# marbl/meryl

Hardware: AMD Instinct MI355X
Metric: distinct k-mers counted/sec (whole node) (higher is better)
Workload: dtype u64; 1 GPU; meryl count k=21 on synthetic short reads: 66666667 x 150 bp reads per GPU (10.00 Gbp per GPU, 30x of a 333333334 bp genome, 0.5% substitutions, 0.01% N), inputs resident in HBM; k=21, reads_per_gpu=66666667, bases_per_gpu=10066666717, n_distinct=1181289506, parallelism=1 GPU, transport=none (one GPU), n_instances=8648488363, w_prefix=18

## Files before the change

### meryl_amd/build.py

```python
import os
import shutil
import subprocess
import sys

HERE = os.path.dirname(os.path.abspath(__file__))
CSRC = os.path.join(HERE, "csrc")
LIB = os.path.join(HERE, "libmeryl_gpu_count.so")
SOURCES = ["mgc_kmer.hip", "mgc_sort.hip", "mgc_scan.hip", "mgc_finish.hip", "mgc_misc.hip", "mgc_parse.hip",
           "mgc_encode.hip", "mgc_decode.hip", "mgc_merge.hip", "mgc_merge_many.hip", "mgc_lookup.hip", "mgc_filter.hip", "mgc_import.hip", "mgc_analyze.hip", "mgc_value_hist.hip",
           "mgc_api.cpp", "mgc_textfile.cpp", "mgc_import.cpp", "mgc_analyze.cpp", "mgc_count.cpp", "mgc_stream.cpp", "mgc_eval.cpp", "mgc_runs.cpp", "mgc_node.cpp", "meryl_db.cpp", "meryl_seq.cpp"]
HEADERS = ["mgc_device.h", "mgc_common.hpp", "mdb_layout.h", "mdb_statistics.hpp", "mgc_session.hpp", "mgc_clock.hpp", "mgc_chunk_ring.hpp", "mgc_bgzf.hpp", "mgc_runs.hpp", "mgc_lookup_dev.hpp", "mgc_import_dev.hpp", "mgc_analyze_dev.hpp", "mgc_label.hpp", "mgc_selector.hpp", "mgc_value.hpp", "mgc_route.hpp",
           os.path.join("..", "..", "include", "meryl_gpu_count.h"),
           os.path.join("..", "..", "include", "meryl_db.h"), os.path.join("..", "..", "include", "meryl_seq.h"),
           os.path.join("..", "..", "include", "meryl_lookup.h"), os.path.join("..", "..", "include", "meryl_import.h"),
           os.path.join("..", "..", "include", "meryl_analyze.h")]
OBJDIR = os.path.join(HERE, "build")
CFLAGS = ["--offload-arch=gfx950", "-O3", "-std=c++17", "-fPIC", "-pthread", "-Wall", "-Wno-unused-function"]
LFLAGS = ["--offload-arch=gfx950", "-shared", "-fPIC", "-pthread", "-no-hip-rt"]


def hipcc():
    for cand in (os.environ.get("HIPCC"), shutil.which("hipcc"), "/opt/rocm/bin/hipcc"):
        if cand and os.path.exists(cand):
            return cand
    raise RuntimeError("hipcc not found: the native library cannot be built")


def _sources():
    return [f for f in SOURCES if os.path.exists(os.path.join(CSRC, f))]


def _header_mtime():
    deps = [os.path.join(CSRC, f) for f in HEADERS if os.path.exists(os.path.join(CSRC, f))]
    deps.append(os.path.abspath(__file__))
    return max(os.path.getmtime(d) for d in deps)


def _obj(f):
    return os.path.join(OBJDIR, f + ".o")


def _stale_objects(force=False):
    ht = _header_mtime()
    out = []
    for f in _sources():
        o = _obj(f)
        if force or not os.path.exists(o) or os.path.getmtime(o) < max(os.path.getmtime(os.path.join(CSRC, f)), ht):
            out.append(f)
    return out


def _stale():
    if not os.path.exists(LIB) or _stale_objects():
        return True
    t = os.path.getmtime(LIB)
    return any(os.path.getmtime(_obj(f)) > t for f in _sources())


CLI = os.path.join(HERE, "bin", "meryl")
LOOKUP_CLI = os.path.join(HERE, "bin", "meryl-lookup")
IMPORT_CLI = os.path.join(HERE, "bin", "meryl-import")
ANALYZE_CLI = os.path.join(HERE, "bin", "meryl-analyze")


def _build_front_end(source, out, force, verbose):
    src = os.path.join(CSRC, source)
    if (not force and os.path.exists(out) and os.path.getmtime(out) >= os.path.getmtime(src)
            and os.path.getmtime(out) >= os.path.getmtime(LIB)):
        return out
    os.makedirs(os.path.dirname(out), exist_ok=True)
    rocm_lib = os.path.join(os.environ.get("ROCM_PATH", "/opt/rocm"), "lib")
    tmp = "%s.tmp%d" % (out, os.getpid())
    cmd = [hipcc(), "-O2", "-std=c++17", "-pthread", src, "-o", tmp, "-L" + HERE, "-lmeryl_gpu_count",
           "-Wl,-rpath,$ORIGIN/..", "-L" + rocm_lib, "-lamdhip64", "-Wl,-rpath," + rocm_lib, "-lz"]
    if verbose:
        print(" ".join(cmd), file=sys.stderr)
    subprocess.check_call(cmd)
    os.replace(tmp, out)
    return out


def build_cli(force=False, verbose=False):
    return _build_front_end("meryl_main.cpp", CLI, force, verbose)


def build_lookup_cli(force=False, verbose=False):
    return _build_front_end("meryl_lookup_main.cpp", LOOKUP_CLI, force, verbose)


def build_import_cli(force=False, verbose=False):
    return _build_front_end("meryl_import_main.cpp", IMPORT_CLI, force, verbose)


def build_analyze_cli(force=False, verbose=False):
    return _build_front_end("meryl_analyze_main.cpp", ANALYZE_CLI, force, verbose)


def build(force=False, verbose=False):
    if not force and not _stale():
        build_cli(False, verbose)
        build_lookup_cli(False, verbose)
        build_import_cli(False, verbose)
        build_analyze_cli(False, verbose)
        return LIB
    os.makedirs(OBJDIR, exist_ok=True)
    todo = _stale_objects(force)
    procs = []
    for f in todo:
        tmp = "%s.tmp%d" % (_obj(f), os.getpid())
        cmd = [hipcc()] + CFLAGS + ["-c", os.path.join(CSRC, f), "-o", tmp]
        if verbose:
            print(" ".join(cmd), file=sys.stderr)
        procs.append((f, tmp, cmd, subprocess.Popen(cmd)))
    failed = []
    for f, tmp, cmd, p in procs:
        if p.wait() != 0:
            failed.append(f)
        else:
            os.replace(tmp, _obj(f))
    if failed:
        raise subprocess.CalledProcessError(1, "hipcc -c " + " ".join(failed))
    tmp = "%s.tmp%d" % (LIB, os.getpid())
    cmd = [hipcc()] + LFLAGS + ["-o", tmp] + [_obj(f) for f in _sources()] + ["-lz"]
    if verbose:
        print(" ".join(cmd), file=sys.stderr)
    subprocess.check_call(cmd)
    os.replace(tmp, LIB)
    build_cli(True, verbose)
    build_lookup_cli(True, verbose)
    build_import_cli(True, verbose)
    build_analyze_cli(True, verbose)
    return LIB


if __name__ == "__main__":
    print(build(force="--force" in sys.argv, verbose=True))
```

### meryl_amd/csrc/mgc_api.cpp

```cpp
#include "../../include/meryl_gpu_count.h"
#include "mgc_device.h"
#include "mgc_session.hpp"
#include "mgc_runs.hpp"
#include "mgc_selector.hpp"
#include "mgc_value.hpp"

#include <algorithm>
#include <cstdio>
#include <cstdlib>
#include <cstring>
#include <map>
#include <string>
#include <thread>
#include <vector>

namespace mgc {
std::string &thread_last_error() {
  thread_local std::string e;
  return e;
}

Switches read_switches() {
  Switches sw;
  auto off = [](const char *n) { const char *e = getenv(n); return e && e[0] == '0'; };
  auto on1 = [](const char *n) { const char *e = getenv(n); return e && e[0] == '1'; };
  auto num = [](const char *n, uint64_t d) { const char *e = getenv(n); return (e && *e) ? strtoull(e, nullptr, 10) : d; };
  sw.fine_hist = !off("MGC_FINE_HIST"); sw.hpc_msd = !off("MGC_HPC_MSD"); sw.hpc_digits = !off("MGC_HPC_DIGITS");
  sw.const_k = !off("MGC_KMER_CONST_K"); sw.narrow = !off("MGC_NARROW"); sw.wide_msd = !off("MGC_WIDE_MSD");
  sw.group_pipe = !off("MGC_GROUP_PIPE"); sw.soa5 = !off("MGC_SOA5"); sw.k96 = !off("MGC_K96"); sw.finish = !off("MGC_FINISH");
  sw.nolist = on1("MGC_FINISH_NOLIST");
  sw.finish_trace = getenv("MGC_FINISH_TRACE") != nullptr; sw.group_dbg = getenv("MGC_GROUP_DBG") != nullptr; sw.hash_dbg = getenv("MGC_HASH_DBG") != nullptr;
  { const char *e = getenv("MGC_HASH_MULTI"); sw.hash_multi = (e && *e) ? atoi(e) : -1; }
  { const char *e = getenv("MGC_HASH_STREAM"); sw.hash_stream = (e && *e) ? atoi(e) : -1; }
  sw.min_top = (uint32_t)num("MGC_FINISH_MIN_TOP", 0);
  sw.finish_target = num("MGC_FINISH_TARGET", 0);
  sw.stream_max = num("MGC_STREAM_MAX", (uint64_t)1 << 22);
  sw.bucket_bases = num("MGC_BUCKET_BASES", 0);
  sw.huge_streams = (uint32_t)num("MGC_HUGE_STREAMS", 4);
  sw.huge_slices = !off("MGC_HUGE_SLICES");
  sw.pass_stagger = (uint32_t)num("MGC_PASS_STAGGER", 0);
  return sw;
}
}
using mgc::set_err;

namespace {


uint64_t number_of_bits64(uint64_t v) {
  uint64_t b = 0;
  while (v) { b++; v >>= 1; }
  return b;
}

uint64_t expected_simple_size(uint32_t k, uint64_t n_est, uint32_t suffix_len) {
  if (2 * k - 2 * suffix_len > 42) return UINT64_MAX;
  const uint64_t low_bits  = 16;
  const uint64_t n_entries = (uint64_t)1 << (2 * k - 2 * suffix_len);
  const uint64_t exp_max   = (uint64_t)(0.004 * (double)n_est);
  const uint64_t exp_bits  = number_of_bits64(exp_max) + 1;
  const uint64_t extra     = (exp_bits < low_bits) ? 0 : (exp_bits - low_bits);
  return (n_entries * low_bits + n_entries * extra) / 8;
}

void best_prefix_size(const mgc_count_config &c, uint64_t n_est, uint64_t mem_allowed, uint32_t *best,
                      uint64_t *mem_used) {
  const uint32_t k = c.k;
  const uint32_t seg_bits = c.page_size * 8, seg_bytes = c.page_size;
  *best = 0;
  *mem_used = UINT64_MAX;
  for (uint32_t wp = 1; wp < 2 * k - 1; wp++) {
    const uint64_t n_prefix = (uint64_t)1 << wp;
    const uint64_t kpp = n_est / n_prefix + 1;
    const uint64_t kps = seg_bits / (2 * k - wp);
    const uint64_t spp = kpp / kps + 1;
    if (wp + number_of_bits64(spp) + number_of_bits64(seg_bytes) >= 64) break;
    const uint64_t struct_mem = (uint64_t)c.sizeof_count_array * n_prefix + 8 * n_prefix * spp;
    const uint64_t data_min   = n_prefix * seg_bytes;
    const uint64_t total      = struct_mem + n_prefix * spp * seg_bytes;
    if (struct_mem + data_min > mem_allowed) break;
    if ((wp > 9) && (total + (uint64_t)16 * wp * 1024 * 1024 < *mem_used)) {
      *mem_used = total;
      *best = wp;
    }
    if (total > (uint64_t)16 * *mem_used) break;
  }
}

}

extern "C" uint32_t mgc_version(void) { return (0u << 16) | 3u; }

extern "C" int mgc_configure_counting(mgc_count_config *c) {
  if (!c) return MGC_EINVAL;
  if (c->k == 0 || c->k > 64) {
    set_err(nullptr, "ERROR: Kmer size not supplied with modifier k=<kmer-size>.");
    return MGC_EINVAL;
  }
  if (c->mode < 0 || c->mode > 2) return MGC_EINVAL;
  if (c->page_size == 0) c->page_size = 4096;
  if (c->sizeof_count_array == 0) c->sizeof_count_array = 3232;

  c->use_simple = 0; c->w_prefix = 0; c->n_prefix = 0; c->w_data = 0; c->n_batches = 1; c->memory_used = 0;

  const uint64_t mem_simple = expected_simple_size(c->k, c->n_kmers_estimate, c->count_suffix_length);
  uint64_t mem_complex = UINT64_MAX;
  uint32_t best = 0, n_batches = 1;

  if (c->k > 5) {
    for (n_batches = 1; mem_complex > c->memory_allowed; n_batches++) {
      best_prefix_size(*c, c->n_kmers_estimate / n_batches, c->memory_allowed, &best, &mem_complex);
      if (n_batches > (1u << 20)) {
        set_err(nullptr, "configureCounting: no prefix size fits in %lu bytes", (unsigned long)c->memory_allowed);
        return MGC_EINVAL;
      }
    }
    c->w_prefix = best;
    c->n_prefix = (uint64_t)1 << best;
    c->w_data   = 2 * c->k - best;
  }
  if ((mem_simple < mem_complex) && (mem_simple < c->memory_allowed)) {
    c->use_simple = 1; c->memory_used = mem_simple;
  } else {
    c->use_simple = 0; c->memory_used = mem_complex;
  }
  if (c->count_suffix_length > 0) { c->use_simple = 1; c->memory_used = mem_simple; }
  c->n_batches = n_batches;
  return MGC_OK;
}

extern "C" int mgc_format_configured_line(const mgc_count_config *c, char *buf, size_t buflen) {
  if (!c || !buf) return MGC_EINVAL;
  const uint64_t m = (c->memory_used < c->memory_allowed) ? c->memory_used : c->memory_allowed;
  snprintf(buf, buflen, "Configured %s mode for %.3f GB memory per batch, and up to %u batch%s.",
           c->use_simple ? "simple" : "complex", m / 1024.0 / 1024.0 / 1024.0, c->n_batches,
           (c->n_batches == 1) ? "" : "es");
  return MGC_OK;
}

namespace {
int hip_rc(hipError_t e, const char *what) {
  if (e == hipSuccess) return MGC_OK;
  set_err(nullptr, "%s: %s", what, hipGetErrorString(e));
  return (e == hipErrorOutOfMemory) ? MGC_ENOMEM : MGC_EHIP;
}
bool key_args_ok(uint32_t k, int mode, uint32_t bucket_bits) {
  if (k == 0 || k > 64) { set_err(nullptr, "k=%u out of range (1..64)", k); return false; }
  if (mode < 0 || mode > 2) { set_err(nullptr, "bad mode %d", mode); return false; }
  if (bucket_bits > MGC_MAX_BUCKET_BITS || bucket_bits > 2 * k) { set_err(nullptr, "bad bucket_bits %u", bucket_bits); return false; }
  return true;
}
}

extern "C" size_t mgc_dev_partition_workspace_bytes(uint32_t bucket_bits) {
  return mgc::kp_workspace_bytes(bucket_bits);
}

extern "C" int mgc_dev_kmer_histogram(const uint8_t *d_bases, uint64_t n_bases, uint32_t k, int mode,
                                      uint32_t bucket_bits, uint64_t *d_bucket_counts, void *d_ws, size_t ws_bytes,
                                      void *stream) {
  if (!key_args_ok(k, mode, bucket_bits)) return MGC_EINVAL;
  if ((!d_bases && n_bases) || !d_bucket_counts || !d_ws || ws_bytes < mgc::kp_workspace_bytes(bucket_bits)) return MGC_EINVAL;
  return hip_rc(mgc::launch_kmer_histogram(d_bases, n_bases, k, mode, bucket_bits, d_bucket_counts, d_ws,
                                           (hipStream_t)stream), "kmer_histogram");
}

extern "C" int mgc_dev_kmer_partition(const uint8_t *d_bases, uint64_t n_bases, uint32_t k, int mode,
                                      uint32_t bucket_bits, const uint64_t *d_bucket_starts, void *d_keys,
                                      void *d_ws, size_t ws_bytes, void *stream) {
  if (!key_args_ok(k, mode, bucket_bits)) return MGC_EINVAL;
  if ((!d_bases && n_bases) || !d_bucket_starts || !d_ws || ws_bytes < mgc::kp_workspace_bytes(bucket_bits)) return MGC_EINVAL;
  return hip_rc(mgc::launch_kmer_partition(d_bases, n_bases, k, mode, bucket_bits, d_bucket_starts, d_keys, d_ws,
                                           (hipStream_t)stream), "kmer_partition");
}

extern "C" int mgc_dev_kmer_histogram_fine(const uint8_t *d_bases, uint64_t n_bases, uint32_t k, int mode, uint32_t bucket_bits,
                                           uint64_t *d_bucket_counts, uint64_t *d_fine_hist, void *d_ws, size_t ws_bytes, void *stream) {
  if (!key_args_ok(k, mode, bucket_bits) || !mgc::kmer_histogram_fine_bits_ok(k, bucket_bits)) return MGC_EINVAL;
  if ((!d_bases && n_bases) || !d_bucket_counts || !d_fine_hist || !d_ws || ws_bytes < mgc::kp_workspace_bytes(bucket_bits)) return MGC_EINVAL;
  const mgc::Switches sw = mgc::read_switches();
  return hip_rc(mgc::launch_kmer_histogram_fine(d_bases, n_bases, k, mode, d_bucket_counts, d_fine_hist, d_ws, (hipStream_t)stream,
                                                sw.const_k, bucket_bits), "kmer_histogram_fine");
}

extern "C" size_t mgc_dev_sort_workspace_bytes(uint64_t n) { return mgc::sort_workspace_bytes(n) + 256; }

static int dev_radix_passes(void *d_keys, void *d_alt, uint64_t n, uint32_t key_words, uint32_t begin_bit, uint32_t end_bit, void *d_ws,
                           size_t ws_bytes, int *result_in_alt, void *stream, bool group);

extern "C" int mgc_dev_radix_sort(void *d_keys, void *d_alt, uint64_t n, uint32_t key_words, uint32_t begin_bit,
                                  uint32_t end_bit, void *d_ws, size_t ws_bytes, int *result_in_alt, void *stream) {
  return dev_radix_passes(d_keys, d_alt, n, key_words, begin_bit, end_bit, d_ws, ws_bytes, result_in_alt, stream, false);
}
extern "C" int mgc_dev_radix_group(void *d_keys, void *d_alt, uint64_t n, uint32_t key_words, uint32_t begin_bit,
                                   uint32_t end_bit, void *d_ws, size_t ws_bytes, int *result_in_alt, void *stream) {
  return dev_radix_passes(d_keys, d_alt, n, key_words, begin_bit, end_bit, d_ws, ws_bytes, result_in_alt, stream, true);
}

static int dev_radix_passes(void *d_keys, void *d_alt, uint64_t n, uint32_t key_words, uint32_t begin_bit, uint32_t end_bit, void *d_ws,
                           size_t ws_bytes, int *result_in_alt, void *stream, bool group) {
  if (!result_in_alt || begin_bit > end_bit || (key_words != 1 && key_words != 2) || end_bit > 64 * key_words) return MGC_EINVAL;
  *result_in_alt = 0;
  if (n == 0 || begin_bit == end_bit) return MGC_OK;
  if (!d_keys || !d_alt || !d_ws || ws_bytes < mgc::sort_workspace_bytes(n) + 256) return MGC_EINVAL;
  mgc::SortPlan plan;
  mgc::make_sort_plan(begin_bit, end_bit, &plan);
  if (group) plan.mode = 3;
  uint32_t *d_err = reinterpret_cast<uint32_t *>(reinterpret_cast<unsigned char *>(d_ws) + mgc::sort_workspace_bytes(n));
  hipStream_t st = (hipStream_t)stream;
  hipError_t e = hipMemsetAsync(d_err, 0, 4, st);
  if (e != hipSuccess) return hip_rc(e, "radix_sort memset");
  e = mgc::launch_radix_sort(d_keys, d_alt, n, key_words, plan, d_ws, ws_bytes - 256, d_err, result_in_alt, st, nullptr);
  if (e != hipSuccess) return hip_rc(e, "radix_sort");
  uint32_t h_err = 0;
  e = hipMemcpyAsync(&h_err, d_err, 4, hipMemcpyDeviceToHost, st);
  if (e == hipSuccess) e = hipStreamSynchronize(st);
  if (e != hipSuccess) return hip_rc(e, "radix_sort sync");
  if (h_err) { set_err(nullptr, "radix sort look-back timed out"); return MGC_ETIMEOUT; }
  return MGC_OK;
}

extern "C" size_t mgc_dev_rle_workspace_bytes(uint64_t n) { return mgc::rle_workspace_bytes(n); }

extern "C" int mgc_dev_rle_count(const void *d_sorted, uint64_t n, uint32_t key_words, void *d_ws, size_t ws_bytes,
                                 uint64_t *n_distinct, void *stream) {
  if (!n_distinct || !d_ws || ws_bytes < mgc::rle_workspace_bytes(n) || (!d_sorted && n) ||
      (key_words != 1 && key_words != 2)) return MGC_EINVAL;
  hipError_t e = mgc::launch_rle_count(d_sorted, n, key_words, d_ws, (hipStream_t)stream);
  if (e != hipSuccess) return hip_rc(e, "rle_count");
  return hip_rc(mgc::rle_read_total(d_ws, n_distinct, (hipStream_t)stream), "rle_count sync");
}

extern "C" int mgc_dev_rle_emit(const void *d_sorted, uint64_t n, uint32_t key_words, void *d_ws, size_t ws_bytes,
                                void *d_unique, uint32_t *d_counts, void *stream) {
  if (!d_ws || ws_bytes < mgc::rle_workspace_bytes(n) || (n && (!d_sorted || !d_unique || !d_counts)) ||
      (key_words != 1 && key_words != 2)) return MGC_EINVAL;
  return hip_rc(mgc::launch_rle_emit(d_sorted, n, key_words, d_ws, d_unique, d_counts, (hipStream_t)stream), "rle_emit");
}

extern "C" uint32_t mgc_dev_value_hist_listed_bins(void) { return mgc::value_hist_small_bins(); }

extern "C" int mgc_dev_value_hist_listed(const uint32_t *d_values, uint64_t n, uint64_t *d_hist, uint32_t *d_big, uint64_t big_cap, void *stream,
                                         uint64_t *n_pairs, uint64_t *n_listed) {
  if ((n && !d_values) || !d_hist || !d_big || big_cap < n || !n_pairs || !n_listed) { set_err(nullptr, "mgc_dev_value_hist_listed: bad arguments"); return MGC_EINVAL; }
  hipStream_t st = (hipStream_t)stream;
  const uint32_t nsmall = mgc::value_hist_small_bins();
  std::vector<uint64_t> h_hist(nsmall + 1);
  std::map<uint64_t, uint64_t> acc;
#define VL_TRY(expr) do { hipError_t e__ = (expr); if (e__ != hipSuccess) {                                         \
    set_err(nullptr, "mgc_dev_value_hist_listed: %s -> %s", #expr, hipGetErrorString(e__)); return MGC_EHIP; } } while (0)
  VL_TRY(hipMemsetAsync(d_hist, 0, 8 * (nsmall + 1), st));
  VL_TRY(mgc::launch_value_hist(d_values, n, d_hist, d_big, big_cap, d_hist + nsmall, st));
  VL_TRY(hipMemcpyAsync(h_hist.data(), d_hist, 8 * (nsmall + 1), hipMemcpyDeviceToHost, st));
  VL_TRY(hipStreamSynchronize(st));
  std::vector<uint32_t> big(h_hist[nsmall]);
  if (!big.empty()) VL_TRY(hipMemcpy(big.data(), d_big, 4 * big.size(), hipMemcpyDeviceToHost));
#undef VL_TRY
  for (uint32_t v = 0; v < nsmall; v++) if (h_hist[v]) acc[v] += h_hist[v];
  for (uint32_t v : big) acc[v]++;
  *n_pairs = acc.size();
  *n_listed = big.size();
  return MGC_OK;
}

extern "C" int mgc_dev_block_offsets(const void *d_unique, uint64_t n_distinct, uint32_t key_words, uint32_t w_data,
                                     uint64_t n_prefix, uint64_t *d_block_start, void *stream) {
  if (!d_block_start || (key_words != 1 && key_words != 2) || w_data >= 64 * key_words || (n_distinct && !d_unique))
    return MGC_EINVAL;
  return hip_rc(mgc::launch_block_offsets(d_unique, n_distinct, key_words, w_data, n_prefix, d_block_start,
                                          (hipStream_t)stream), "block_offsets");
}

extern "C" size_t mgc_dev_merge_workspace_bytes(uint64_t na, uint64_t nb) { return mgc::merge_workspace_bytes(na, nb); }

extern "C" int mgc_dev_merge_count(const void *dA, uint64_t na, const void *dB, uint64_t nb, uint32_t key_words, int op, void *d_ws,
                                   size_t ws_bytes, uint64_t *n_out, void *stream) {
  if (!n_out || !d_ws || ws_bytes < mgc::merge_workspace_bytes(na, nb) || (na && !dA) || (nb && !dB) ||
      (key_words != 1 && key_words != 2) || op < 0 || op > MGC_MERGE_SYMMETRIC_DIFFERENCE || op == MGC_MERGE_SUBTRACT) return MGC_EINVAL;
  hipError_t e = mgc::launch_merge_count(dA, na, dB, nb, key_words, op, d_ws, (hipStream_t)stream);
  if (e != hipSuccess) return hip_rc(e, "merge_count");
  return hip_rc(mgc::merge_read_total(d_ws, n_out, (hipStream_t)stream), "merge_count sync");
}

extern "C" int mgc_dev_merge_count_values(const void *dA, const uint32_t *cA, uint64_t na, const void *dB, const uint32_t *cB, uint64_t nb,
                                          uint32_t key_words, int op, void *d_ws, size_t ws_bytes, uint64_t *n_out, void *stream) {
  if (!n_out || !d_ws || ws_bytes < mgc::merge_workspace_bytes(na, nb) || (na && (!dA || !cA)) || (nb && (!dB || !cB)) ||
      (key_words != 1 && key_words != 2) || op < 0 || op > MGC_MERGE_SYMMETRIC_DIFFERENCE) return MGC_EINVAL;
  hipError_t e = mgc::launch_merge_count(dA, na, dB, nb, key_words, op, d_ws, (hipStream_t)stream, cA, cB);
  if (e != hipSuccess) return hip_rc(e, "merge_count");
  return hip_rc(mgc::merge_read_total(d_ws, n_out, (hipStream_t)stream), "merge_count sync");
}

extern "C" size_t mgc_dev_select_workspace_bytes(uint64_t n) { return mgc::select_workspace_bytes(n); }

extern "C" int mgc_dev_select_count(const void *d_keys, const uint32_t *d_values, uint64_t n, uint32_t key_words, int value_op, uint64_t constant,
                                    void *d_ws, size_t ws_bytes, uint64_t *n_out, void *stream) {
  if (!n_out || !d_ws || ws_bytes < mgc::select_workspace_bytes(n) || (n && (!d_keys || !d_values)) || (key_words != 1 && key_words != 2) ||
      value_op < 0 || value_op > MGC_VALUE_MODULO) return MGC_EINVAL;
  hipError_t e = mgc::launch_select(false, mgc::SelectInput{d_keys, d_values, nullptr, nullptr, n, key_words}, value_op, constant, mgc::PassRule(), d_ws, nullptr, nullptr,
                                    (hipStream_t)stream);
  if (e != hipSuccess) return hip_rc(e, "select_count");
  return hip_rc(mgc::merge_read_total(d_ws, n_out, (hipStream_t)stream), "select_count sync");
}

extern "C" int mgc_dev_select_emit(const void *d_keys, const uint32_t *d_values, uint64_t n, uint32_t key_words, int value_op, uint64_t constant,
                                   void *d_ws, size_t ws_bytes, void *d_keys_out, uint32_t *d_values_out, void *stream) {
  if (!d_ws || ws_bytes < mgc::select_workspace_bytes(n) || (n && (!d_keys || !d_values)) || (key_words != 1 && key_words != 2) ||
      value_op < 0 || value_op > MGC_VALUE_MODULO) return MGC_EINVAL;
  return hip_rc(mgc::launch_select(true, mgc::SelectInput{d_keys, d_values, nullptr, nullptr, n, key_words}, value_op, constant, mgc::PassRule(), d_ws, d_keys_out,
                                   d_values_out, (hipStream_t)stream), "select_emit");
}

extern "C" int mgc_dev_merge_emit(const void *dA, const uint32_t *cA, uint64_t na, const void *dB, const uint32_t *cB, uint64_t nb,
                                  uint32_t key_words, int op, void *d_ws, size_t ws_bytes, void *d_keys_out, uint32_t *d_counts_out,
                                  void *stream) {
  if (!d_ws || ws_bytes < mgc::merge_workspace_bytes(na, nb) || (na && (!dA || !cA)) || (nb && (!dB || !cB)) ||
      (key_words != 1 && key_words != 2) || op < 0 || op > MGC_MERGE_SYMMETRIC_DIFFERENCE) return MGC_EINVAL;
  return hip_rc(mgc::launch_merge_emit(dA, cA, na, dB, cB, nb, key_words, op, d_ws, d_keys_out, d_counts_out, (hipStream_t)stream),
                "merge_emit");
}

extern "C" uint32_t mgc_dev_merge_many_tile(uint32_t key_words) { return mgc::merge_many_tile(key_words); }

static bool merge_many_args_ok(const void *const *d_keys, const uint32_t *const *d_values, const uint64_t *n, uint32_t n_inputs,
                               uint32_t key_words, int op, uint32_t min_inputs = 2) {
  if (!d_keys || !d_values || !n || n_inputs < min_inputs || n_inputs > MGC_MERGE_MANY_MAX || (key_words != 1 && key_words != 2) ||
      op < MGC_MERGE_UNION_SUM || op > MGC_MERGE_UNION) return false;
  for (uint32_t i = 0; i < n_inputs; i++)
    if ((n[i] && (!d_keys[i] || !d_values[i])) || (n[i] >> 32)) return false;
  return true;
}
// ... 910 lines not shown
```

### meryl_amd/csrc/mgc_count.cpp

```cpp
#include "mgc_session.hpp"

#include <algorithm>
#include <deque>
#include <vector>

#define TRY(expr) do { const int rc__ = (expr); if (rc__ != MGC_OK) return rc__; } while (0)

namespace {
using S = mgc_session;

struct DevBuf {
  void *p = nullptr;
  ~DevBuf() { if (p) (void)hipFree(p); }
  hipError_t alloc(size_t bytes) { return hipMalloc(&p, bytes ? bytes : 256); }
};

struct StageTimer {
  bool on;
  hipStream_t st;
  hipEvent_t ev[MGC_NUM_STAGES][2];
  bool used[MGC_NUM_STAGES];
  StageTimer(bool enable, hipStream_t s) : on(enable), st(s) {
    for (int i = 0; i < MGC_NUM_STAGES; i++) {
      used[i] = false;
      if (on) { (void)hipEventCreate(&ev[i][0]); (void)hipEventCreate(&ev[i][1]); }
    }
  }
  ~StageTimer() {
    if (on) for (int i = 0; i < MGC_NUM_STAGES; i++) { (void)hipEventDestroy(ev[i][0]); (void)hipEventDestroy(ev[i][1]); }
  }
  void begin(int i) { if (on) { (void)hipEventRecord(ev[i][0], st); used[i] = true; } }
  void end(int i)   { if (on) (void)hipEventRecord(ev[i][1], st); }
};

enum class Group : uint8_t {
  NONE,
  SORT,
  NARROW,
  WIDE,
};

struct FilePlan {
  uint64_t size = 0, start = 0;
  uint32_t top = 0;
  uint32_t top_str = 0;
  mgc::SortPlan sp{};
  Group kind = Group::NONE;
  bool hpc = false;
  bool hpc_stream = false;
  bool hpc_cand = false;
  bool hpc_mixed = false;
  bool stream = false;
  bool k96 = false;
  bool msd_ok = true;
  uint32_t tr_a = 0, tr_b = 0;
  uint64_t gbase = 0, sbase = 0, slots = 0;
  size_t nws_off = 0;
  uint32_t *cnt = nullptr;
  uint64_t maxsub = 0, nlarge = 0, nzcount = 0;
  bool fallback = false;
  uint32_t passes = 0; bool narrowed = false, k96_passes = false;
  uint64_t ngf() const { return size ? (uint64_t)1 << top : 0; }
};

uint32_t plan_bucket_bits(const mgc_count_config &c, const mgc::Switches &sw, uint64_t n_bases) {
  const uint64_t per_bucket = sw.bucket_bases ? sw.bucket_bases
                                              : (c.homopoly_compress ? 60000000ull : 180000000ull);
  const uint32_t step = c.homopoly_compress ? 2u : 1u;
  uint32_t bits = MGC_NUM_FILES_BITS;
  while (bits + step <= MGC_MAX_BUCKET_BITS && bits + step <= 2 * c.k && (n_bases >> bits) > per_bucket) bits += step;
  return bits;
}

struct CountPlan {
  const mgc_count_config &c;
  const mgc::Switches &sw;
  mgc_profile &prof;
  uint32_t kw, bucket_bits, nb, rem_bits, fine_bits;
  bool fine = false;
  bool fine_hpc = false;
  uint64_t max_bucket = 0, ng_total = 0, ns_total = 0;
  uint64_t target = 0, cap = 0, starget = 0;
  bool stream_on = false, hpc_ok = false, hpc_stream_ok = false, hpc_mixed_ok = false;
  std::vector<FilePlan> files;

  CountPlan(const mgc_count_config &c_, const mgc::Switches &sw_, mgc_profile &prof_, uint32_t kw_, uint32_t bucket_bits_)
      : c(c_), sw(sw_), prof(prof_), kw(kw_), bucket_bits(bucket_bits_), nb(1u << bucket_bits_), rem_bits(2 * c_.k - bucket_bits_),
        fine_bits(15u - bucket_bits_), files(nb) {}

  mgc::SortPlan group_plan(uint32_t low) const {
    mgc::SortPlan p;
    mgc::make_sort_plan(low, rem_bits, &p);
    if (p.mode == 0) p.mode = 3;
    return p;
  }
  void fit_split(FilePlan &x) const {
    mgc::SortPlan &fp = x.sp;
    if (!fine || fp.num_passes != 2 || fp.hpc || fp.pass_bits[1] <= fine_bits) return;
    const uint32_t t = fp.pass_bits[0] + fp.pass_bits[1];
    if (t - fine_bits > 9) { x.msd_ok = false; return; }
    fp.pass_bits[1] = fine_bits; fp.pass_bits[0] = t - fine_bits;
    fp.pass_shift[1] = fp.pass_shift[0] + fp.pass_bits[0];
  }

  void init() {
    target = mgc::finish_target_for(kw, sw); cap = mgc::finish_capacity_for(kw);
    stream_on = sw.hash_stream != 0 && kw == 1 && !c.homopoly_compress;
    starget = mgc::finish_stream_target(sw);
    hpc_ok = sw.hpc_digits && c.homopoly_compress && (rem_bits % 2 == 0) && bucket_bits >= 2;
    hpc_stream_ok = hpc_ok && sw.hash_stream != 0 && sw.hash_stream != 2 && kw == 1 && fine_hpc && nb <= 256 && sw.wide_msd &&
                    rem_bits >= 20 + 32 && mgc::finish_stream_ok(kw, rem_bits - 20, false);
    hpc_mixed_ok = hpc_stream_ok && rem_bits >= 18 + 32 && mgc::finish_stream_ok(kw, rem_bits - 18, false) && mgc::finish_uses_hash(kw, rem_bits - 18);
  }

  uint32_t plan_top(FilePlan &x) const {
    uint32_t t = 0;
    if (hpc_ok && x.size > target) {
      if (x.size <= 243ull * target && rem_bits >= 10) t = 10;
      else if (x.size <= 59049ull * target && rem_bits >= 20) t = 20;
      else if (hpc_stream_ok && x.size <= 59049ull * starget && x.size < (1ull << 30)) { t = 20; x.hpc_stream = true; }
      if (t == 20 && sw.hash_stream == 1 && hpc_stream_ok && x.size < (1ull << 30)) x.hpc_stream = true;
      if (t) x.hpc = true;
    }
    if (!x.hpc) {
      while (t < rem_bits && t < 26 && (x.size >> t) > target) t++;
      if (sw.min_top) { const uint32_t m = sw.min_top; if (x.size && t < m) t = m < rem_bits ? m : rem_bits; }
      if (stream_on && x.size) {
        uint32_t ts = 0;
        while (ts < rem_bits && ts < 26 && (x.size >> ts) > starget) ts++;
        if (sw.min_top) { const uint32_t m = sw.min_top; if (ts < m) ts = m < rem_bits ? m : rem_bits; }
        x.top_str = ts;
      }
    }
    if (c.homopoly_compress && t && !x.hpc) {
      const double scale = 1.0 / (1.0 - 0.2075);
      const uint32_t tc = (uint32_t)((double)t * scale + 0.5);
      t = tc < rem_bits ? (tc < 26 ? tc : 26) : rem_bits;
    }
    return t;
  }

  void plan_hpc_kind(FilePlan &x) {
    mgc::make_hpc_group_plan(rem_bits - x.top, x.top / 10, &x.sp);
    const bool wide = fine_hpc && nb <= 256 && x.top == 20 && (kw == 2 || rem_bits - x.top >= 32) &&
                      mgc::finish_uses_hash(kw, rem_bits - x.top) && mgc::sort_plan_wide_msd(x.sp, x.size, sw.wide_msd);
    x.kind = wide ? Group::WIDE : Group::SORT;
    if (x.hpc_stream && wide) { x.stream = true; prof.stream_files++; }
    else if (hpc_stream_ok && wide && x.top == 20 && x.size < (1ull << 30)) x.hpc_cand = true;
    if ((x.hpc_cand || (x.stream && sw.hash_stream == 1)) && hpc_mixed_ok && x.size >= 19683ull * (starget * 3 / 10) &&
        x.size <= 19683ull * starget) {
      mgc::SortPlan mp;
      mgc::make_hpc_mixed_plan(rem_bits - 18, &mp);
      x.hpc_mixed = mgc::sort_plan_wide_msd(mp, x.size, sw.wide_msd);
      if (x.hpc_mixed && sw.hash_stream == 1) { take_coarser(x); x.hpc_mixed = x.hpc_cand = false; }
    }
  }

  void plan_bit_kind(FilePlan &x) {
    x.sp = group_plan(rem_bits - x.top);
    fit_split(x);
    const uint32_t low = rem_bits - x.top;
    if (low < 32 && mgc::finish_uses_hash(kw, low) && mgc::sort_plan_narrows(x.sp, x.size, kw, sw.narrow)) x.kind = Group::NARROW;
    else if (fine && nb <= 256 && x.msd_ok && mgc::finish_uses_hash(kw, low) && mgc::sort_plan_wide_msd(x.sp, x.size, sw.wide_msd)) x.kind = Group::WIDE;
    else x.kind = Group::SORT;
    if (!x.top_str) return;
    const bool narrow = x.kind == Group::NARROW;
    uint32_t ts = x.top_str;
    const uint32_t t = x.top, max_low = narrow ? 20u : 52u;
    if (rem_bits - ts > max_low) ts = rem_bits - max_low;
    bool ok = ts >= 1 && ts <= t && ts <= 18 && (ts < t || sw.hash_stream == 1) && (narrow || (x.kind == Group::WIDE && kw == 1 && sw.hash_stream != 2)) &&
              x.size < (1ull << 32) && mgc::finish_stream_ok(kw, rem_bits - ts, narrow) && mgc::finish_uses_hash(kw, rem_bits - ts);
    if (ok) {
      const mgc::SortPlan sp = group_plan(rem_bits - ts);
      if (narrow) ok = mgc::sort_plan_narrows(sp, x.size, kw, sw.narrow);
      else {
        const bool split_ok = !(fine && sp.num_passes == 2 && sp.pass_bits[1] > fine_bits && ts - fine_bits > 9);
        ok = split_ok && mgc::sort_plan_wide_msd(sp, x.size, sw.wide_msd);
      }
    }
    x.top_str = ok ? ts : 0;
  }

  void plan_files() {
    init();
    for (FilePlan &x : files) {
      x.top = plan_top(x);
      if (x.size == 0 || x.top == 0) continue;
      if (x.hpc) plan_hpc_kind(x);
      else plan_bit_kind(x);
    }
    for (FilePlan &x : files) {
      x.slots = x.ngf();
      x.gbase = ng_total; x.sbase = ns_total;
      ng_total += x.slots;
      ns_total += x.slots ? x.slots + 1 : 0;
    }
  }

  void take_coarser(FilePlan &x) {
    if (!x.stream) { x.stream = true; prof.stream_files++; }
    if (x.top_str) {
      x.top = x.top_str;
      x.sp = group_plan(rem_bits - x.top);
      x.msd_ok = true;
      fit_split(x);
    } else if (x.hpc_mixed) {
      x.top = 18;
      mgc::make_hpc_mixed_plan(rem_bits - 18, &x.sp);
      prof.hpc_mixed_files++;
    }
  }

  int choose_probe() {
    bool any_cand = false;
    for (const FilePlan &x : files) any_cand = any_cand || x.top_str != 0 || x.hpc_cand;
    if (!any_cand) return -1;
    if (sw.hash_stream == 1) {
      for (FilePlan &x : files) if (x.top_str) take_coarser(x);
      return -1;
    }
    int probe = -1;
    uint64_t best = ~0ull;
    for (uint32_t b = 0; b < nb; b++)
      if (files[b].size >= max_bucket / 16 && files[b].size >= 4096 && files[b].size < best) { best = files[b].size; probe = (int)b; }
    return probe;
  }
  void apply_probe(uint32_t probe) {
    for (uint32_t b = 0; b < nb; b++)
      if (b != probe && (files[b].top_str || (files[b].hpc_cand && !files[b].stream))) take_coarser(files[b]);
  }

  uint32_t soa_mask(bool plain_input) const {
    bool soa = sw.soa5 && plain_input && kw == 1 && nb == 64 && fine && rem_bits > 32 && rem_bits <= 40;
    for (const FilePlan &x : files) if (x.size && !(x.kind == Group::NARROW && x.top)) soa = false;
    return soa ? (1u << (rem_bits - 32)) - 1u : 0u;
  }
  bool k96_layout(bool plain_input) {
    if (!(sw.k96 && plain_input && kw == 2 && nb == 64 && fine && rem_bits <= 96 && !c.homopoly_compress)) return false;
    bool any = false;
    for (FilePlan &x : files) if (x.size && x.kind == Group::WIDE && x.top) { x.k96 = true; any = true; prof.k96_files++; }
    return any;
  }
};

struct Count {
  mgc_session *s;
  const mgc::CountInput &in;
  hipStream_t st;
  const mgc_count_config &c;
  const mgc::Switches &sw;
  mgc_profile &prof;
  const uint32_t k, kw, bucket_bits, nb, rem_bits;
  const size_t kbytes;
  CountPlan plan;
  StageTimer tm;
  hipEvent_t ev_all[2] = {nullptr, nullptr};

  const uint8_t *d_bases;
  uint64_t n_bases, N = 0, nd = 0;
  void *part_ws = nullptr, *sort_ws = nullptr, *rle_ws = nullptr;
  uint64_t *d_counts64 = nullptr, *d_starts = nullptr;
  std::vector<uint64_t> h_meta;
  const uint64_t *d_fine = nullptr, *d_fine_hpc = nullptr;
  mgc::SortPlan full{};
  bool use_finish;
  unsigned char *X = nullptr, *Y = nullptr;
  size_t sort_ws_bytes = 0;
  uint32_t *d_err = nullptr;
  uint32_t soa_hi_mask = 0;
  static constexpr uint32_t ev_per_file = 2 * 16;
  std::vector<hipEvent_t> pass_ev;
  uint32_t sort_launch_groups = 0;

  int probe = -1;
  uint64_t *d_substart = nullptr, *d_group = nullptr, *d_stats = nullptr, *d_retrycnt = nullptr;
  uint32_t *d_large = nullptr, *d_nz = nullptr;
  const size_t hdr_bytes = mgc::sort_header_bytes();
  unsigned char *d_nws = nullptr, *d_nhdrs = nullptr;
  std::deque<DevBuf> cnt_extra;
  bool fork_huge = false, forked = false, need_join = false;
  static constexpr int NH = 1 + S::HUGE_EXTRA;
  hipStream_t hstream[NH] = {};
  unsigned char *halt[NH] = {};
  void *hws[NH] = {nullptr, nullptr, nullptr, nullptr};
  size_t hws_bytes = 0;
  int n_huge_streams = 1, huge_next = 0;
  std::vector<std::pair<hipEvent_t, hipEvent_t>> fin_ev;
  uint64_t fin_keys = 0, fin_in_bytes = 0; bool fin_narrow = false;

  Count(mgc_session *s_, const mgc::CountInput &in_, uint32_t bucket_bits_)
      : s(s_), in(in_), st(s_->stream), c(s_->cfg), sw(s_->sw), prof(s_->prof), k(c.k), kw(s_->key_words), bucket_bits(bucket_bits_),
        nb(1u << bucket_bits_), rem_bits(2 * c.k - bucket_bits_), kbytes(sizeof(uint64_t) * kw), plan(c, sw, s_->prof, kw, bucket_bits_),
        tm(s_->profiling, s_->stream), d_bases(s_->d_bases), n_bases(s_->n_bases), h_meta(2 * (size_t)nb, 0), use_finish(sw.finish) {}

  void *seg(uint32_t b) const { return X + kbytes * plan.files[b].start; }
  uint32_t low(const FilePlan &x) const { return rem_bits - x.top; }
  const uint32_t *nz_list(const FilePlan &x) const { return (4 * x.nzcount < 3 * x.ngf() && !sw.nolist) ? d_nz + x.gbase : nullptr; }
  bool msd_file(const FilePlan &x) const {
    return d_fine_hpc ? x.kind == Group::WIDE : (x.kind == Group::NARROW || x.kind == Group::WIDE) && x.msd_ok;
  }
  mgc::FinishFile finish_desc(uint32_t b, bool stream, hipStream_t fst, int hsel) const;
  void take_stats(uint32_t b) {
    const uint64_t *h = s->h_stats + 3 * (size_t)b;
    plan.files[b].maxsub = h[0]; plan.files[b].nlarge = h[1]; plan.files[b].nzcount = h[2];
  }

  int run();
  int compress_bases(); int histogram(); int buffers(); int partition(bool soa, bool k96);
  int count_full();
  int count_finish(); int finish_buffers(); int prepare_headers(); int narrow_prepare(int only, int skip);
  int probe_file(); int group_file(uint32_t b); int stats_file(uint32_t b); int group_all();
  int huge_setup(); int huge_sync_all(); int huge_join_all();
  int finish_file(uint32_t b); int oversized_streams(uint32_t b, bool *stream); int widen_back(uint32_t b, bool *unordered);
  int count_file(uint32_t b, bool stream); int fallback_file(uint32_t b, bool unordered);
  int trace_slices(); int retry(); int scan_pack(); int pack_file(uint32_t b); void finish_profile();
  int block_offsets(); void collect_profile();
};

int Count::compress_bases() {
  if (!c.homopoly_compress || !n_bases || in.keys) return MGC_OK;
  HIP_TRY(s, s->ensure(S::B_HPC, n_bases));
  HIP_TRY(s, s->ensure(S::B_HPC_WS, mgc::hpc_workspace_bytes(n_bases)));
  uint8_t *d_hpc = reinterpret_cast<uint8_t *>(s->buf[S::B_HPC].p);
  void *hws_ = s->buf[S::B_HPC_WS].p;
  HIP_TRY(s, mgc::launch_homopoly_compress(d_bases, n_bases, d_hpc, hws_, st));
  uint64_t n_out = 0;
  HIP_TRY(s, hipMemcpyAsync(&n_out, hws_, sizeof(uint64_t), hipMemcpyDeviceToHost, st));
  HIP_TRY(s, hipStreamSynchronize(st));
  d_bases = d_hpc;
  n_bases = n_out;
  return MGC_OK;
}

int Count::histogram() {
  HIP_TRY(s, s->ensure(S::B_PART_WS, mgc::kp_workspace_bytes(bucket_bits)));
  HIP_TRY(s, s->ensure(S::B_META, sizeof(uint64_t) * nb * 3));
  part_ws = s->buf[S::B_PART_WS].p;
  d_counts64 = reinterpret_cast<uint64_t *>(s->buf[S::B_META].p);
  d_starts = d_counts64 + nb;
  std::vector<uint64_t> h_counts(nb);
  const bool wide_msd_on = sw.wide_msd && !c.homopoly_compress;
  if (!in.keys) {
    tm.begin(MGC_STAGE_HISTOGRAM);
    if (n_bases >= (1u << 22) && ((kw == 1 && 2 * k - bucket_bits <= 41) || wide_msd_on) && mgc::kmer_histogram_fine_ok(k, bucket_bits, s->sfx_mask, sw)) {
      HIP_TRY(s, s->ensure(S::B_FINE, sizeof(uint64_t) << 15));
      uint64_t *fine = reinterpret_cast<uint64_t *>(s->buf[S::B_FINE].p);
      HIP_TRY(s, mgc::launch_kmer_histogram_fine(d_bases, n_bases, k, c.mode, d_counts64, fine, part_ws, st, sw.const_k));
      d_fine = fine;
    } else if (c.homopoly_compress && n_bases >= (1u << 22) && (2 * k - bucket_bits) % 2 == 0 && 2 * k - bucket_bits >= 20 &&
               sw.hpc_digits && mgc::kmer_histogram_hpc_ok(k, bucket_bits, s->sfx_mask, sw)) {
      HIP_TRY(s, s->ensure(S::B_FINE, sizeof(uint64_t) * std::max<size_t>((size_t)1 << 15, mgc::kmer_histogram_hpc_entries(bucket_bits))));
      uint64_t *fine = reinterpret_cast<uint64_t *>(s->buf[S::B_FINE].p);
      HIP_TRY(s, mgc::launch_kmer_histogram_hpc(d_bases, n_bases, k, c.mode, bucket_bits, d_counts64, fine, part_ws, st, sw.const_k));
      d_fine_hpc = fine;
    } else
    HIP_TRY(s, mgc::launch_kmer_histogram(d_bases, n_bases, k, c.mode, bucket_bits, d_counts64, part_ws, st, s->sfx_mask, s->sfx_test));
    tm.end(MGC_STAGE_HISTOGRAM);
    prof.stage_launches[MGC_STAGE_HISTOGRAM] = 1;
    HIP_TRY(s, hipMemcpyAsync(h_counts.data(), d_counts64, sizeof(uint64_t) * nb, hipMemcpyDeviceToHost, st));
    HIP_TRY(s, hipStreamSynchronize(st));
  } else {
    memcpy(h_counts.data(), in.counts, sizeof(uint64_t) * nb);
    uint64_t n_ext = 0;
    for (uint32_t b = 0; b < nb; b++) n_ext += h_counts[b];
    if (in.fine && sw.fine_hist && bucket_bits <= 8 && n_ext >= (1u << 22) && s->sfx_mask == 0 && !c.homopoly_compress &&
        2 * k >= 15 + 2 && ((kw == 1 && 2 * k - bucket_bits <= 41) || wide_msd_on))
      d_fine = in.fine;
  }
  memset(s->file_instances, 0, sizeof(s->file_instances));
  for (uint32_t b = 0; b < nb; b++) {
    plan.files[b].size = h_counts[b];
    plan.files[b].start = h_meta[b] = N;
    N += h_counts[b];
    plan.max_bucket = std::max(plan.max_bucket, h_counts[b]);
    s->file_instances[b >> (bucket_bits - MGC_NUM_FILES_BITS)] += h_counts[b];
  }
  s->n_instances = N;
  plan.fine = d_fine != nullptr;
  plan.fine_hpc = d_fine_hpc != nullptr;
  return MGC_OK;
}

int Count::buffers() {
  mgc::make_sort_plan(0, rem_bits, &full);
  const bool odd = !use_finish && (full.num_passes & 1u) != 0;
  if (!in.keys) HIP_TRY(s, s->ensure(S::B_X, kbytes * N));
  HIP_TRY(s, s->ensure(S::B_Y, kbytes * (odd ? N : plan.max_bucket)));
  X = in.keys ? reinterpret_cast<unsigned char *>(in.keys) : reinterpret_cast<unsigned char *>(s->buf[S::B_X].p);
  Y = reinterpret_cast<unsigned char *>(s->buf[S::B_Y].p);
  sort_ws_bytes = mgc::sort_workspace_bytes(plan.max_bucket) + 256;
  HIP_TRY(s, s->ensure(S::B_SORT_WS, sort_ws_bytes));
  sort_ws = s->buf[S::B_SORT_WS].p;
  d_err = reinterpret_cast<uint32_t *>(reinterpret_cast<unsigned char *>(sort_ws) + sort_ws_bytes - 256);
  HIP_TRY(s, hipMemsetAsync(d_err, 0, 32, st));
  if (s->profiling) {
    pass_ev.resize((size_t)nb * ev_per_file);
    for (auto &e : pass_ev) (void)hipEventCreate(&e);
  }
  return MGC_OK;
}

int Count::partition(bool soa, bool k96) {
  if (in.keys) return MGC_OK;
  HIP_TRY(s, hipMemcpyAsync(d_starts, h_meta.data(), sizeof(uint64_t) * nb, hipMemcpyHostToDevice, st));
  uint64_t *d_k96flags = d_starts + nb;
  if (k96) HIP_TRY(s, hipMemcpyAsync(d_k96flags, h_meta.data() + nb, sizeof(uint64_t) * nb, hipMemcpyHostToDevice, st));
  tm.begin(MGC_STAGE_PARTITION);
  HIP_TRY(s, mgc::launch_kmer_partition(d_bases, n_bases, k, c.mode, bucket_bits, d_starts, (void *)X, part_ws, st,
                                        s->sfx_mask, s->sfx_test, k96 ? d_k96flags : (soa ? d_counts64 : nullptr), sw.const_k));
  tm.end(MGC_STAGE_PARTITION);
  prof.hist_bytes = n_bases;
  prof.partition_bytes = n_bases;
  for (uint32_t b = 0; b < nb; b++) prof.partition_bytes += plan.files[b].size * (soa ? 5u : ((k96 && plan.files[b].k96) ? 12u : (uint64_t)kbytes));
  prof.stage_launches[MGC_STAGE_PARTITION] = 2;
  return MGC_OK;
}

int Count::count_full() {
  TRY(partition(false, false));
  const bool odd = (full.num_passes & 1u) != 0;
  tm.begin(MGC_STAGE_SORT);
  for (uint32_t b = 0; b < nb; b++) {
    FilePlan &x = plan.files[b];
    if (x.size == 0) continue;
    void *alt = odd ? (void *)(Y + kbytes * x.start) : (void *)Y;
    int in_alt = 0;
    hipEvent_t *pe = s->profiling ? &pass_ev[(size_t)b * ev_per_file] : nullptr;
    HIP_TRY(s, mgc::launch_radix_sort(seg(b), alt, x.size, kw, full, sort_ws, sort_ws_bytes - 256, d_err, &in_alt, st, pe));
    x.passes = full.num_passes;
    sort_launch_groups++;
  }
  tm.end(MGC_STAGE_SORT);
  void *d_sorted = odd ? (void *)Y : (void *)X;

  HIP_TRY(s, s->ensure(S::B_RLE_WS, mgc::rle_workspace_bytes(N)));
  rle_ws = s->buf[S::B_RLE_WS].p;
  tm.begin(MGC_STAGE_RLE);
  HIP_TRY(s, mgc::launch_rle_count(d_sorted, N, kw, rle_ws, st));
  HIP_TRY(s, mgc::rle_read_total(rle_ws, &nd, st));
  s->n_distinct = nd;
  HIP_TRY(s, s->ensure(S::B_UNIQUE, kbytes * nd));
  HIP_TRY(s, s->ensure(S::B_COUNTS, sizeof(uint32_t) * nd));
  s->d_unique = s->buf[S::B_UNIQUE].p;
  s->d_counts = reinterpret_cast<uint32_t *>(s->buf[S::B_COUNTS].p);
  HIP_TRY(s, mgc::launch_rle_emit(d_sorted, N, kw, rle_ws, s->d_unique, s->d_counts, st));
  tm.end(MGC_STAGE_RLE);
  prof.stage_launches[MGC_STAGE_RLE] = 3;
  return MGC_OK;
}

int Count::finish_buffers() {
  const uint64_t ng_total = plan.ng_total;
  HIP_TRY(s, s->ensure(S::B_SUBSTART, sizeof(uint64_t) * (plan.ns_total + 1)));
  HIP_TRY(s, s->ensure(S::B_GROUPS, sizeof(uint64_t) * (ng_total + 2 + 3 * (uint64_t)nb)));
  HIP_TRY(s, s->ensure(S::B_LARGE, sizeof(uint32_t) * (ng_total + 1)));
  HIP_TRY(s, s->ensure(S::B_NONEMPTY, sizeof(uint32_t) * (ng_total + 1) + sizeof(uint64_t) * 2 * ((uint64_t)nb + 1)));
  HIP_TRY(s, s->ensure(S::B_GSCAN, mgc::finish_scan_scratch_bytes(ng_total + 1)));
  HIP_TRY(s, s->ensure(S::B_RLE_WS, mgc::rle_workspace_bytes(plan.max_bucket)));
  d_substart = reinterpret_cast<uint64_t *>(s->buf[S::B_SUBSTART].p);
  d_group    = reinterpret_cast<uint64_t *>(s->buf[S::B_GROUPS].p);
  d_stats    = d_group + ng_total + 1;
  d_large    = reinterpret_cast<uint32_t *>(s->buf[S::B_LARGE].p);
  d_retrycnt = reinterpret_cast<uint64_t *>(s->buf[S::B_NONEMPTY].p) + nb + 1;
  d_nz       = reinterpret_cast<uint32_t *>(d_retrycnt + nb + 1);
  HIP_TRY(s, hipMemsetAsync(s->buf[S::B_NONEMPTY].p, 0, sizeof(uint64_t) * 2 * ((size_t)nb + 1), st));
  HIP_TRY(s, hipMemsetAsync(d_group, 0, sizeof(uint64_t) * (ng_total + 1 + 3 * (size_t)nb), st));
  rle_ws = s->buf[S::B_RLE_WS].p;
  return MGC_OK;
}

int Count::prepare_headers() {
  if ((!d_fine && !d_fine_hpc) || nb > 256) return MGC_OK;
  uint64_t on[4] = {0, 0, 0, 0};
  size_t off = 0;
  bool any = false;
  for (uint32_t b = 0; b < nb; b++) {
    FilePlan &x = plan.files[b];
    x.nws_off = off;
    if (!msd_file(x)) continue;
    any = true;
    on[b >> 6] |= 1ull << (b & 63u);
    off += ((x.kind == Group::NARROW ? mgc::narrow_scratch_bytes(x.size) : mgc::wide_scratch_bytes(x.size, kw)) + 255) / 256 * 256;
  }
  if (!any) return MGC_OK;
  HIP_TRY(s, s->ensure(S::B_SORT_HDRS, hdr_bytes * nb));
  HIP_TRY(s, s->ensure(S::B_NARROW_WS, off));
  d_nhdrs = reinterpret_cast<unsigned char *>(s->buf[S::B_SORT_HDRS].p);
  d_nws = reinterpret_cast<unsigned char *>(s->buf[S::B_NARROW_WS].p);
  if (d_fine) TRY(narrow_prepare(probe, -1));
  else HIP_TRY(s, mgc::launch_hpc_prepare(d_fine_hpc, bucket_bits, on, d_nhdrs, st));
  HIP_TRY(s, hipMemsetAsync(d_nws, 0, off, st));
  return MGC_OK;
}

int Count::narrow_prepare(int only, int skip) {
  unsigned char bits_a[256] = {0}, on[256] = {0};
  bool any = false;
  for (uint32_t b = 0; b < nb; b++) {
    if (!msd_file(plan.files[b]) || (only >= 0 && (int)b != only) || (int)b == skip) continue;
    on[b] = 1; bits_a[b] = (unsigned char)plan.files[b].sp.pass_bits[1]; any = true;
  }
  if (any) HIP_TRY(s, mgc::launch_narrow_prepare(d_fine, nb, bits_a, on, d_nhdrs, st));
  return MGC_OK;
}

int Count::group_file(uint32_t b) {
  FilePlan &x = plan.files[b];
  if (x.size == 0) return MGC_OK;
  void *src = seg(b);
  hipEvent_t *pe = s->profiling ? &pass_ev[(size_t)b * ev_per_file] : nullptr;
  switch (x.kind) {
  case Group::NONE:
    return MGC_OK;
  case Group::NARROW: {
    const bool msd = d_nhdrs && d_nws && x.msd_ok;
    HIP_TRY(s, mgc::launch_group_narrow(src, (void *)Y, x.size, x.sp, sort_ws, sort_ws_bytes - 256, d_err, d_substart + x.sbase, st, pe,
                                        msd ? (void *)(d_nhdrs + hdr_bytes * b) : nullptr, msd ? (void *)(d_nws + x.nws_off) : nullptr,
                                        &x.tr_a, &x.tr_b, soa_hi_mask, sw.group_dbg, sw.group_pipe, sw.pass_stagger));
    x.passes = 2;
    x.narrowed = true;
    break;
  }
  case Group::WIDE:
    if (d_nhdrs) {
      HIP_TRY(s, mgc::launch_group_wide(src, (void *)Y, x.size, kw, x.sp, d_err, d_substart + x.sbase, st, pe,
                                        (void *)(d_nhdrs + hdr_bytes * b), (void *)(d_nws + x.nws_off), &x.tr_a, &x.tr_b, x.k96));
      x.passes = 2;
      x.k96_passes = x.k96;
      prof.wide_msd_files++;
      break;
    }
    x.kind = Group::SORT;
    [[fallthrough]];
  case Group::SORT: {
    int in_alt = 0;
    HIP_TRY(s, mgc::launch_radix_sort(src, (void *)Y, x.size, kw, x.sp, sort_ws, sort_ws_bytes - 256, d_err, &in_alt, st, pe));
    if (in_alt) HIP_TRY(s, hipMemcpyAsync(src, Y, kbytes * x.size, hipMemcpyDeviceToDevice, st));
    x.passes = x.sp.num_passes;
    break;
  }
  }
  sort_launch_groups++;
  return MGC_OK;
}

int Count::stats_file(uint32_t b) {
  const FilePlan &x = plan.files[b];
  if (x.size == 0) return MGC_OK;
  uint64_t *ds = d_stats + 3 * (size_t)b;
  if (x.kind == Group::NARROW || x.kind == Group::WIDE)
    HIP_TRY(s, mgc::launch_subbucket_max(d_substart + x.sbase, kw, low(x), x.top, ds, d_large + x.gbase, ds + 1, d_nz + x.gbase, ds + 2, st,
                                         x.stream ? mgc::finish_stream_capacity() : 0));
  else
    HIP_TRY(s, mgc::launch_subbucket_bounds(seg(b), x.size, kw, low(x), x.top, d_substart + x.sbase, ds, d_large + x.gbase, ds + 1,
                                            d_nz + x.gbase, ds + 2, st));
  return MGC_OK;
}

int Count::probe_file() {
  const uint32_t pb = (uint32_t)probe;
  const FilePlan &x = plan.files[pb];
  TRY(group_file(pb));
  TRY(stats_file(pb));
  HIP_TRY(s, hipMemcpyAsync(s->h_stats + 3 * (size_t)pb, d_stats + 3 * (size_t)pb, sizeof(uint64_t) * 3, hipMemcpyDeviceToHost, st));
  HIP_TRY(s, hipStreamSynchronize(st));
  take_stats(pb);
  TRY(finish_file(pb));
  if (need_join) TRY(huge_join_all());
  forked = false;
  uint64_t h_pd = 0;
  HIP_TRY(s, mgc::launch_sum_u64(d_group + x.gbase, x.slots, d_group + plan.ng_total, st));
  HIP_TRY(s, hipMemcpyAsync(&h_pd, d_group + plan.ng_total, sizeof(uint64_t), hipMemcpyDeviceToHost, st));
  HIP_TRY(s, hipStreamSynchronize(st));
  const double ratio = (double)h_pd / (double)x.size;
  prof.probe_ratio = ratio;
  if (sw.finish_trace) fprintf(stderr, "[finish] probe file %u: %llu distinct of %llu k-mers (%.3f): the other files take the %s plan\n", pb,
                               (unsigned long long)h_pd, (unsigned long long)x.size, ratio, ratio <= 0.30 ? "distinct-sized" : "finer");
  if (ratio <= 0.30) plan.apply_probe(pb);
  if (d_fine && nb <= 256 && d_nhdrs) TRY(narrow_prepare(-1, probe));
  return MGC_OK;
}

int Count::group_all() {
  for (uint32_t b = 0; b < nb; b++) if ((int)b != probe) TRY(group_file(b));
  tm.end(MGC_STAGE_SORT);
  tm.begin(MGC_STAGE_RLE);
  for (uint32_t b = 0; b < nb; b++) if ((int)b != probe) TRY(stats_file(b));
  HIP_TRY(s, hipMemcpyAsync(s->h_stats, d_stats, sizeof(uint64_t) * 3 * (size_t)nb, hipMemcpyDeviceToHost, st));
  HIP_TRY(s, hipStreamSynchronize(st));
  for (uint32_t b = 0; b < nb; b++) if ((int)b != probe) take_stats(b);
  return huge_setup();
}

int Count::huge_setup() {
  uint32_t files_gigantic = 0;
  for (uint32_t b = 0; b < nb; b++) if (plan.files[b].size && s->h_stats[3 * (size_t)b + 1] != 0 && s->h_stats[3 * (size_t)b] > 16384) files_gigantic++;
  if (files_gigantic && sw.huge_slices) {
    HIP_TRY(s, s->ensure(S::B_HWS0, hws_bytes));
    hws[0] = s->buf[S::B_HWS0].p;
  }
  const int want = (int)std::min<uint64_t>((uint64_t)sw.huge_streams, (uint64_t)NH);
  if (!fork_huge || want <= 1 || files_gigantic < 2) return MGC_OK;
  for (int i = 1; i < want; i++) {
    if (!s->stream_h[i - 1] && hipStreamCreateWithFlags(&s->stream_h[i - 1], hipStreamNonBlocking) != hipSuccess) { s->stream_h[i - 1] = nullptr; (void)hipGetLastError(); }
    if (!s->stream_h[i - 1]) break;
    const int id = S::B_Y2 + (i - 1);
    HIP_TRY(s, s->ensure(id, kbytes * plan.max_bucket));
    hstream[i] = s->stream_h[i - 1];
    halt[i] = reinterpret_cast<unsigned char *>(s->buf[id].p);
    if (sw.huge_slices) { HIP_TRY(s, s->ensure(S::B_HWS0 + i, hws_bytes)); hws[i] = s->buf[S::B_HWS0 + i].p; }
    n_huge_streams = i + 1;
  }
  return MGC_OK;
}

int Count::huge_sync_all() {
  for (int i = 0; i < n_huge_streams; i++) HIP_TRY(s, hipStreamSynchronize(hstream[i]));
  return MGC_OK;
}

int Count::huge_join_all() {
  for (int i = 0; i < n_huge_streams; i++) {
    HIP_TRY(s, hipEventRecord(s->ev_join, hstream[i]));
    HIP_TRY(s, hipStreamWaitEvent(st, s->ev_join, 0));
  }
  return MGC_OK;
}

int Count::finish_file(uint32_t b) {
  FilePlan &x = plan.files[b];
  x.fallback = false;
  if (x.size == 0) return MGC_OK;
  bool stream = false, unordered = false;
  TRY(oversized_streams(b, &stream));
  if (x.nlarge > 0 && !stream && (x.k96 || x.kind == Group::NARROW)) TRY(widen_back(b, &unordered));
  if (x.kind == Group::WIDE && x.nlarge > 0 && !stream) unordered = true;
  if ((x.maxsub <= plan.cap || stream) && !unordered) return count_file(b, stream);
  return fallback_file(b, unordered);
}

int Count::oversized_streams(uint32_t b, bool *stream) {
  const FilePlan &x = plan.files[b];
  *stream = mgc::finish_uses_hash(kw, low(x)) && x.nlarge > 0;
  if (*stream && x.maxsub > sw.stream_max && kw == 2) {
    *stream = false;
  } else if (*stream && x.maxsub > sw.stream_max) {
    uint32_t h_fail[3] = {0, 0, 0};
    HIP_TRY(s, hipMemsetAsync(d_err + 4, 0, 12, st));
    HIP_TRY(s, mgc::launch_finish_probe(finish_desc(b, true, st, 0), sw.stream_max, d_err + 4));
    HIP_TRY(s, hipMemcpyAsync(h_fail, d_err + 4, 12, hipMemcpyDeviceToHost, st));
    HIP_TRY(s, hipStreamSynchronize(st));
    *stream = (h_fail[0] == 0);
    if (sw.finish_trace)
      fprintf(stderr, "[finish] bucket %u: largest sub-bucket %llu > %llu, up to %u distinct in one: %s\n", b,
              (unsigned long long)x.maxsub, (unsigned long long)sw.stream_max, h_fail[2],
              *stream ? "streamed through the hash tables" : "too many distinct: stable-sort fallback");
  } else if (sw.finish_trace && x.maxsub > plan.cap) {
    fprintf(stderr, "[finish] bucket %u: largest sub-bucket %llu > %llu: %s\n", b, (unsigned long long)x.maxsub,
            (unsigned long long)plan.cap, *stream ? "streamed through the hash tables" : "stable-sort fallback");
  }
  return MGC_OK;
}

int Count::widen_back(uint32_t b, bool *unordered) {
  FilePlan &x = plan.files[b];
  if (need_join) TRY(huge_sync_all());
  forked = false;
  if (x.k96) {
    const unsigned __int128 fb = (unsigned __int128)b << rem_bits;
    HIP_TRY(s, mgc::launch_widen_k96(seg(b), x.size, (uint64_t)fb, (uint64_t)(fb >> 64), (void *)Y, st));
  } else {
    HIP_TRY(s, mgc::launch_widen_groups(seg(b), d_substart + x.sbase, x.ngf(), (uint64_t)b << rem_bits, low(x), (void *)Y, st, x.tr_a, x.tr_b));
  }
  HIP_TRY(s, hipMemcpyAsync(seg(b), Y, kbytes * x.size, hipMemcpyDeviceToDevice, st));
  if (x.k96) {
    x.k96 = false;
    prof.k96_widened_files++;
    return MGC_OK;
  }
  x.kind = Group::SORT;
  *unordered = x.tr_a != 0;
  if (x.stream) { x.stream = false; *unordered = true; }
  cnt_extra.emplace_back();
  HIP_TRY(s, cnt_extra.back().alloc(sizeof(uint32_t) * x.size));
  x.cnt = reinterpret_cast<uint32_t *>(cnt_extra.back().p);
  return MGC_OK;
}

mgc::FinishFile Count::finish_desc(uint32_t b, bool stream, hipStream_t fst, int hsel) const {
  const FilePlan &x = plan.files[b];
  mgc::FinishFile f;
  f.keys = seg(b); f.alt = halt[hsel];
  f.layout = x.kind == Group::NARROW ? mgc::FinishKeys::NARROW32 : x.k96 ? mgc::FinishKeys::K96 : kw == 2 ? mgc::FinishKeys::WHOLE16 : mgc::FinishKeys::WHOLE8;
  f.starts = d_substart + x.sbase; f.ng = x.ngf(); f.low_bits = low(x); f.tr_a = x.tr_a; f.tr_b = x.tr_b;
  f.n_keys = x.size; f.max_sub = x.maxsub;
  f.cnt_tmp = x.cnt; f.group_distinct = d_group + x.gbase;
  f.large_list = d_large + x.gbase; f.n_large = x.nlarge; f.stream = stream;
  f.nonempty_list = nz_list(x); f.nonempty_count = d_stats + 3 * (size_t)b + 2;
  f.retry_list = x.stream ? d_large + x.gbase + x.nlarge : d_nz + x.gbase; f.retry_count = d_retrycnt + b;
  f.stream_cap = x.stream ? mgc::finish_stream_capacity() : 0;
  f.huge_ws = hws[hsel]; f.huge_ws_bytes = hws_bytes; f.huge_ws_keys = plan.max_bucket; f.d_error = d_err;
  f.st = fst; f.st_huge = hstream[hsel];
  f.hash_multi = sw.hash_multi; f.hash_dbg = sw.hash_dbg;
  return f;
}

int Count::count_file(uint32_t b, bool stream) {
  const FilePlan &x = plan.files[b];
  const bool on_second = fork_huge && (b & 1u);
  if ((stream || on_second) && fork_huge && !forked) {
    HIP_TRY(s, hipEventRecord(s->ev_fork, st));
    for (int i = 0; i < n_huge_streams; i++) HIP_TRY(s, hipStreamWaitEvent(hstream[i], s->ev_fork, 0));
    forked = need_join = true;
  }
  hipStream_t fst = on_second ? s->stream2 : st;
// ... 225 lines not shown
```

### meryl_amd/csrc/mgc_device.h

```cpp
#pragma once

#include <hip/hip_runtime.h>
#include <stddef.h>
#include <stdint.h>
#include "mgc_label.hpp"
#include "../../include/meryl_gpu_count.h"

namespace mgc {

struct Switches {
  bool fine_hist = true;
  bool hpc_msd = true;
  bool hpc_digits = true;
  bool const_k = true;
  bool narrow = true;
  bool wide_msd = true;
  bool soa5 = true;
  bool group_pipe = true;
  bool k96 = true;
  bool finish = true;
  bool nolist = false;
  bool finish_trace = false;
  bool group_dbg = false;
  uint32_t pass_stagger = 0;
  bool hash_dbg = false;
  int  hash_multi = -1;
  int  hash_stream = -1;
  uint32_t min_top = 0;
  uint64_t finish_target = 0;
  uint64_t stream_max = (uint64_t)1 << 22;
  bool     huge_slices = true;
  uint32_t huge_streams = 4;
  uint64_t bucket_bases = 0;
};
Switches read_switches();



constexpr int      KP_BLOCK       = 256;
constexpr int      KP_ITEMS       = 16;
constexpr int      KP_TILE        = KP_BLOCK * KP_ITEMS;
constexpr int      KP_MAX_BUCKETS = 1024;

uint32_t kp_grid_size(uint64_t n_bases, uint32_t bucket_bits);
size_t   kp_workspace_bytes(uint32_t bucket_bits);

bool       kmer_histogram_fine_ok(uint32_t k, uint32_t bucket_bits, uint64_t sfx_mask, const Switches &sw);
bool       kmer_histogram_hpc_ok(uint32_t k, uint32_t bucket_bits, uint64_t sfx_mask, const Switches &sw);
uint32_t   kmer_histogram_hpc_entries(uint32_t bucket_bits);
hipError_t launch_kmer_histogram_hpc(const uint8_t *d_bases, uint64_t n_bases, uint32_t k, int mode, uint32_t bucket_bits,
                                     uint64_t *d_bucket_counts, uint64_t *d_fine_hist, void *d_ws, hipStream_t st, bool const_k = true );
hipError_t launch_kmer_histogram_fine(const uint8_t *d_bases, uint64_t n_bases, uint32_t k, int mode, uint64_t *d_bucket_counts,
                                      uint64_t *d_fine_hist, void *d_ws, hipStream_t st, bool const_k = true ,
                                      uint32_t bucket_bits = 6 );
bool       kmer_histogram_fine_bits_ok(uint32_t k, uint32_t bucket_bits);
hipError_t launch_kmer_histogram(const uint8_t *d_bases, uint64_t n_bases, uint32_t k, int mode,
                                 uint32_t bucket_bits, uint64_t *d_bucket_counts, void *d_ws, hipStream_t st,
                                 uint64_t sfx_mask = 0, uint64_t sfx_test = 0);
hipError_t launch_kmer_partition(const uint8_t *d_bases, uint64_t n_bases, uint32_t k, int mode,
                                 uint32_t bucket_bits, const uint64_t *d_bucket_starts, void *d_keys,
                                 void *d_ws, hipStream_t st, uint64_t sfx_mask = 0, uint64_t sfx_test = 0,
                                 const uint64_t *d_soa_counts = nullptr ,
                                 bool const_k = true );

struct SortPlan {
  uint32_t radix_bits;
  uint32_t block;
  uint32_t kpt;
  uint32_t tile;
  uint32_t mode;
  uint32_t hpc;
  uint32_t num_passes;
  uint32_t pass_shift[16];
  uint32_t pass_bits[16];
};

void   make_sort_plan(uint32_t begin_bit, uint32_t end_bit, SortPlan *plan);
void   make_hpc_group_plan(uint32_t low_bit, uint32_t passes, SortPlan *plan);
void   make_hpc_mixed_plan(uint32_t low_bit, SortPlan *plan);
size_t sort_workspace_bytes(uint64_t n);

hipError_t launch_radix_sort(void *d_keys, void *d_alt, uint64_t n, uint32_t key_words, const SortPlan &plan,
                             void *d_ws, size_t ws_bytes, uint32_t *d_error, int *result_in_alt,
                             hipStream_t st, hipEvent_t *pass_events );
size_t     sort_header_bytes();
bool       sort_plan_narrows(const SortPlan &plan, uint64_t n, uint32_t key_words, bool on = true );
size_t     narrow_scratch_bytes(uint64_t n);
hipError_t launch_narrow_prepare(const uint64_t *d_fine, uint32_t nb, const unsigned char *bits_a, const unsigned char *on, void *d_hdrs,
                                 hipStream_t st);
hipError_t launch_group_narrow(void *d_keys, void *d_alt, uint64_t n, const SortPlan &plan, void *d_ws, size_t ws_bytes,
                               uint32_t *d_error, uint64_t *d_sub_starts, hipStream_t st, hipEvent_t *pass_events ,
                               void *d_prepared, void *d_scratch, uint32_t *tr_a, uint32_t *tr_b,
                               uint32_t soa_hi_mask = 0 ,
                               bool group_dbg = false ,
                               bool pipe = true ,
                               uint32_t stagger = 0 );

bool       sort_plan_wide_msd(const SortPlan &plan, uint64_t n, bool on = true );
hipError_t launch_hpc_prepare(const uint64_t *d_fine_hpc, uint32_t bucket_bits, const uint64_t on[4], void *d_hdrs, hipStream_t st);
size_t     wide_scratch_bytes(uint64_t n, uint32_t key_words);
hipError_t launch_group_wide(void *d_keys, void *d_alt, uint64_t n, uint32_t key_words, const SortPlan &plan, uint32_t *d_error,
                             uint64_t *d_sub_starts, hipStream_t st, hipEvent_t *pass_events , void *d_prepared,
                             void *d_scratch, uint32_t *tr_a, uint32_t *tr_b,
                             bool k96 = false );

size_t     rle_workspace_bytes(uint64_t n);
hipError_t launch_rle_count(const void *d_sorted, uint64_t n, uint32_t key_words, void *d_ws, hipStream_t st);
hipError_t rle_read_total(const void *d_ws, uint64_t *n_distinct, hipStream_t st);
hipError_t launch_rle_emit(const void *d_sorted, uint64_t n, uint32_t key_words, void *d_ws, void *d_unique,
                           uint32_t *d_counts, hipStream_t st, const uint64_t *d_out_base = nullptr);

uint64_t   finish_capacity_for(uint32_t key_words);
uint64_t   finish_target_for(uint32_t key_words, const Switches &sw);
bool       finish_stream_ok(uint32_t key_words, uint32_t low_bits, bool narrow = true);
uint64_t   finish_stream_capacity();
uint64_t   finish_stream_target(const Switches &sw);
uint64_t   finish_stream_distinct();
hipError_t launch_subbucket_bounds(const void *d_keys, uint64_t n, uint32_t key_words, uint32_t low, uint32_t top_bits,
                                   uint64_t *d_starts , uint64_t *d_max ,
                                   uint32_t *d_large_list ,
                                   uint64_t *d_large_count ,
                                   uint32_t *d_nonempty_list , uint64_t *d_nonempty_count ,
                                   hipStream_t st);
hipError_t launch_subbucket_max(const uint64_t *d_starts, uint32_t key_words, uint32_t low, uint32_t top_bits, uint64_t *d_max,
                                uint32_t *d_large_list, uint64_t *d_large_count, uint32_t *d_nonempty_list, uint64_t *d_nonempty_count,
                                hipStream_t st, uint64_t small_cap = 0 );
bool       finish_uses_hash(uint32_t key_words, uint32_t low_bits);
enum class FinishKeys : uint32_t {
  WHOLE8,
  NARROW32,
  K96,
  WHOLE16,
};
struct FinishFile {
  void *keys = nullptr;
  void *alt = nullptr;
  FinishKeys layout = FinishKeys::WHOLE8;
  const uint64_t *starts = nullptr;
  uint64_t ng = 0;
  uint32_t low_bits = 0;
  uint32_t tr_a = 0, tr_b = 0;
  uint64_t n_keys = 0;
  uint64_t max_sub = 0;
  uint32_t *cnt_tmp = nullptr;
  uint64_t *group_distinct = nullptr;
  const uint32_t *large_list = nullptr;
  uint64_t n_large = 0;
  bool stream = false;
  const uint32_t *nonempty_list = nullptr;
  const uint64_t *nonempty_count = nullptr;
  uint32_t *retry_list = nullptr;
  uint64_t *retry_count = nullptr;
  uint64_t stream_cap = 0;
  void *huge_ws = nullptr; size_t huge_ws_bytes = 0; uint64_t huge_ws_keys = 0;
  uint32_t *d_error = nullptr;
  hipStream_t st = nullptr;
  hipStream_t st_huge = nullptr;
  int  hash_multi = -1;
  bool hash_dbg = false;
};
hipError_t launch_finish_probe(const FinishFile &f, uint64_t stream_max , uint32_t *d_file_fail);
hipError_t launch_finish_file(const FinishFile &f);
hipError_t launch_finish_retry(const FinishFile &f, uint64_t n_retry);
size_t     finish_huge_workspace_bytes(uint64_t n_keys);
struct HugeTrace { uint32_t cut, slices, dense; };
hipError_t finish_huge_trace(const void *d_ws, uint64_t ws_keys, HugeTrace *out);
size_t     finish_scan_scratch_bytes(uint64_t ng_total);
hipError_t launch_finish_scan(uint64_t *d_group , uint64_t ng_total, void *d_scratch, hipStream_t st);
hipError_t launch_compact_groups(const void *d_keys, uint32_t key_words, const uint32_t *d_cnt_tmp, const uint64_t *d_starts,
                                 const uint64_t *d_offs, uint64_t ng, void *d_out_keys, uint32_t *d_out_counts, hipStream_t st,
                                 uint32_t tr_a = 0, uint32_t tr_b = 0 ,
                                 const uint32_t *d_nonempty_list = nullptr, uint64_t n_nonempty = 0 );
hipError_t launch_compact_groups_narrow(const void *d_keys32, const uint32_t *d_cnt_tmp, const uint64_t *d_starts, const uint64_t *d_offs,
                                        uint64_t ng, uint64_t base, uint32_t low_bits, void *d_out_keys, uint32_t *d_out_counts, hipStream_t st,
                                        uint32_t tr_a, uint32_t tr_b, const uint32_t *d_nonempty_list = nullptr, uint64_t n_nonempty = 0);
hipError_t launch_compact_groups_k96(const void *d_keys96, const uint32_t *d_cnt_tmp, const uint64_t *d_starts, const uint64_t *d_offs,
                                     uint64_t ng, uint64_t base_lo, uint64_t base_hi, void *d_out_keys, uint32_t *d_out_counts, hipStream_t st,
                                     uint32_t tr_a, uint32_t tr_b, const uint32_t *d_nonempty_list = nullptr, uint64_t n_nonempty = 0);
hipError_t launch_widen_k96(const void *d_keys96, uint64_t n, uint64_t base_lo, uint64_t base_hi, void *d_out128, hipStream_t st);
hipError_t launch_widen_groups(const void *d_keys32, const uint64_t *d_starts, uint64_t ng, uint64_t base, uint32_t low_bits, void *d_out64,
                               hipStream_t st, uint32_t tr_a, uint32_t tr_b);
hipError_t launch_store_u64(uint64_t *d_dst, const uint64_t *d_src, hipStream_t st);
hipError_t launch_sum_u64(const uint64_t *d_in, uint64_t n, uint64_t *d_out, hipStream_t st);

hipError_t launch_block_offsets(const void *d_unique, uint64_t n_distinct, uint32_t key_words, uint32_t w_data,
                                uint64_t n_prefix, uint64_t *d_block_start, hipStream_t st);

hipError_t launch_block_offsets_range(const void *d_keys, uint64_t n, uint32_t key_words, uint32_t w_data, uint64_t prefix_begin,
                                      uint64_t n_blocks, uint64_t n_prefix_total, uint64_t *d_rel_start, hipStream_t st);
hipError_t launch_encode_sizes(const void *d_keys, uint32_t key_words, const uint64_t *d_bs, uint64_t n_blocks, uint32_t suffix_size,
                               uint32_t label_size, uint64_t *d_blk_bytes, uint64_t *d_blk_vbase, uint32_t *d_blk_bb, hipStream_t st);
hipError_t launch_encode_chunk(const void *d_keys, const uint32_t *d_counts, uint32_t key_words, const uint64_t *d_bs,
                               const uint64_t *d_blk_pos, const uint64_t *d_blk_vbase, const uint32_t *d_blk_bb,
                               uint64_t b0, uint64_t b1, uint64_t n_kmers_chunk, uint64_t prefix_of_block0,
                               uint32_t suffix_size, uint32_t label_size, uint64_t label, void *d_img, hipStream_t st,
                               const uint64_t *d_labels = nullptr );
uint32_t   value_hist_small_bins();
hipError_t launch_value_hist(const uint32_t *d_counts, uint64_t n, uint64_t *d_hist, uint32_t *d_big_list, uint64_t big_cap,
                             uint64_t *d_big_n, hipStream_t st);

hipError_t launch_decode_blocks(const void *d_file, const void *d_blocks, uint64_t n_blocks, uint32_t suffix_size, uint32_t label_size,
                                uint32_t key_words, void *d_keys, uint32_t *d_counts, uint32_t *d_err, hipStream_t st,
                                uint64_t *d_labels = nullptr );

size_t     merge_workspace_bytes(uint64_t na, uint64_t nb);
hipError_t launch_merge_count(const void *dA, uint64_t na, const void *dB, uint64_t nb, uint32_t key_words, int op, void *d_ws,
                              hipStream_t st, const uint32_t *cA = nullptr, const uint32_t *cB = nullptr);
hipError_t merge_read_total(const void *d_ws, uint64_t *n_out, hipStream_t st);
hipError_t launch_merge_emit(const void *dA, const uint32_t *cA, uint64_t na, const void *dB, const uint32_t *cB, uint64_t nb,
                             uint32_t key_words, int op, void *d_ws, void *d_out_keys, uint32_t *d_out_counts, hipStream_t st);
struct PassRule {
  int       lop = 0;
  uint64_t  lc = 0;
  bool      select = false;
  const ::mgc_select_term *terms = nullptr;
  uint32_t  n_terms = 0, k = 0;
  int       vop = 0;
  uint64_t  vc = 0;
  int       fop = -1;
  uint64_t  fc = 0;
  uint64_t *out_labs = nullptr;
};
struct MergeManyInputs { const void *const *keys; const uint32_t *const *vals; const uint64_t *const *labs; const uint64_t *n; uint32_t count, key_words; };
uint32_t   merge_many_tile(uint32_t key_words);
size_t     merge_many_workspace_bytes(const uint64_t *n, uint32_t n_inputs, uint32_t key_words);
hipError_t launch_merge_many(bool emit, const MergeManyInputs &in, int op, const PassRule &rule, void *d_ws, void *d_out_keys,
                             uint32_t *d_out_vals, hipStream_t st);
struct SelectInput { const void *keys; const uint32_t *vals; const uint32_t *flags; const uint64_t *labs; uint64_t n; uint32_t key_words; };
size_t     select_workspace_bytes(uint64_t n);
hipError_t launch_select(bool emit, const SelectInput &in, int fop, uint64_t constant, const PassRule &rule, void *d_ws, void *d_out_keys,
                         uint32_t *d_out_vals, hipStream_t st);
hipError_t launch_fill_u32(uint32_t *d, uint64_t n, uint32_t v, hipStream_t st);
hipError_t launch_last_breaker(const uint8_t *d_bases, uint64_t n, uint64_t *d_out, hipStream_t st);

size_t     hpc_workspace_bytes(uint64_t n);
hipError_t launch_homopoly_compress(const uint8_t *d_in, uint64_t n, uint8_t *d_out, void *d_ws, hipStream_t st);

size_t     text_parse_state_bytes();
size_t     text_parse_workspace_bytes(uint64_t n);
hipError_t launch_text_parse(const uint8_t *d_text, uint64_t n, int fastq, void *d_state, void *d_ws, uint8_t *d_out, hipStream_t st);
hipError_t launch_text_file_op(void *d_state, uint8_t *d_out, int what, hipStream_t st);
hipError_t launch_text_set_len(void *d_state, uint64_t new_len, int rebase_file, hipStream_t st);

hipError_t launch_synth_reads(uint64_t seed, uint64_t genome_len, uint64_t first_read, uint64_t n_reads,
                              uint32_t read_len, uint32_t sub_rate_ppm, uint32_t n_rate_ppm,
                              uint32_t repeat_ppm, uint32_t repeat_unit, uint32_t repeat_families,
                              uint8_t *d_out, hipStream_t st);

hipError_t warm_kmer(); hipError_t warm_sort(); hipError_t warm_finish(); hipError_t warm_encode(); hipError_t warm_scan();
}
```

### meryl_amd/csrc/mgc_kmer.hip

```cpp
#include "mgc_common.hpp"

namespace mgc {


__device__ __forceinline__ u32 enc4(u32 w) {
  return (((w >> 1) & 0x03030303u) * 0x40100401u) >> 24;
}
__device__ __forceinline__ u32 zero_bytes(u32 x) {
  return ~(((x & 0x7F7F7F7Fu) + 0x7F7F7F7Fu) | x | 0x7F7F7F7Fu);
}
__device__ __forceinline__ u32 inv4(u32 w) {
  const u32 u = w & 0xDFDFDFDFu;
  const u32 ok = zero_bytes(u ^ 0x41414141u) | zero_bytes(u ^ 0x43434343u) |
                 zero_bytes(u ^ 0x47474747u) | zero_bytes(u ^ 0x54545454u);
  const u32 g = ((~ok) & 0x80808080u) >> 7;
  return ((g * 0x08040201u) >> 24) & 0xFu;
}


__device__ __forceinline__ void encode16(uint4 v, u32 &codes, u32 &inval) {
  codes = (enc4(v.x) << 24) | (enc4(v.y) << 16) | (enc4(v.z) << 8) | enc4(v.w);
  inval = (inv4(v.x) << 12) | (inv4(v.y) << 8) | (inv4(v.z) << 4) | inv4(v.w);
}

__device__ __forceinline__ u64 revcomp64(u64 f, u32 key_shift ) {
  u64 x = __brevll(f ^ 0xAAAAAAAAAAAAAAAAull);
  x = ((x >> 1) & 0x5555555555555555ull) | ((x & 0x5555555555555555ull) << 1);
  return x >> key_shift;
}

constexpr int KP_WORDS = KP_TILE / 16 + 4;

__device__ __forceinline__ void kp_stage_tile(const uint8_t *__restrict__ bases, u64 n, u64 tile0, bool aligned,
                                              u32 *s_codes, u32 *s_inval) {
  const u32 t = threadIdx.x;
  {
    u32 c, iv;
    encode16(load16(bases, tile0 + (u64)t * 16, n, aligned), c, iv);
    s_codes[t] = c; s_inval[t] = iv;
  }
  if (t < 4) {
    u32 c, iv;
    encode16(load16(bases, tile0 + (u64)KP_TILE + (u64)t * 16, n, aligned), c, iv);
    s_codes[KP_BLOCK + t] = c; s_inval[KP_BLOCK + t] = iv;
  }
}

__device__ __forceinline__ u32 kp_valid_mask(u64 I, u32 k) {
  u64 X = I;
  u32 c = 1;
  while (2 * c <= k) { X |= X << c; c *= 2; }
  if (c < k) X |= X << (k - c);
  return __brev((u32)(~X >> 48) & 0xFFFFu) >> 16;
}

__device__ __forceinline__ u32 kp_thread_kmers(const u32 *s_codes, const u32 *s_inval, u32 k, int mode,
                                               u64 (&keys)[KP_ITEMS]) {
  const u32 t = threadIdx.x;
  const u64 A = ((u64)s_codes[t] << 32) | (u64)s_codes[t + 1];
  const u64 B = (u64)s_codes[t + 2] << 32;
  const u64 I = ((u64)s_inval[t] << 48) | ((u64)s_inval[t + 1] << 32) | ((u64)s_inval[t + 2] << 16);
  const u32 key_shift = 64 - 2 * k;
  const u32 top_shift = 2 * k - 2;
  u64 r = 0;
#pragma unroll
  for (int j = 0; j < KP_ITEMS; j++) {
    const u64 top = (j == 0) ? A : ((A << (2 * j)) | (B >> (64 - 2 * j)));
    const u64 f   = top >> key_shift;
    if (j == 0) r = revcomp64(f, key_shift);
    else        r = (r >> 2) | ((((f & 3ull) ^ 2ull)) << top_shift);
    u64 key;
    if      (mode == 1) key = f;
    else if (mode == 2) key = r;
    else                key = (f < r) ? f : r;
    keys[j] = key;
  }
  return kp_valid_mask(I, k);
}

__device__ __forceinline__ u32 kp_thread_buckets(const u32 *s_codes, const u32 *s_inval, u32 k, int mode, u32 bucket_bits,
                                                 u32 (&bk)[KP_ITEMS], const u32 t = threadIdx.x) {
  const u64 A = ((u64)s_codes[t] << 32) | (u64)s_codes[t + 1];
  const u64 B = (u64)s_codes[t + 2] << 32;
  const u64 I = ((u64)s_inval[t] << 48) | ((u64)s_inval[t + 1] << 32) | ((u64)s_inval[t + 2] << 16);
  const u32 m  = (bucket_bits + 1) / 2;
  const u32 z0 = k - m;
  const u64 Z  = (z0 == 0) ? A : ((A << (2 * z0)) | (B >> (64 - 2 * z0)));
  const u64 RC = revcomp64(Z, 0);
  const u64 mmask = (1ull << (2 * m)) - 1ull;
  const u32 odd = 2 * m - bucket_bits;
#pragma unroll
  for (int j = 0; j < KP_ITEMS; j++) {
    const u32 ft = (u32)(((j == 0) ? A : (A << (2 * j))) >> (64 - bucket_bits));
    const u32 rt = (u32)((RC >> (2 * j)) & mmask) >> odd;
    bk[j] = (mode == 1) ? ft : (mode == 2) ? rt : (ft < rt ? ft : rt);
  }
  return kp_valid_mask(I, k);
}

__device__ __forceinline__ u32 kp_thread_buckets_wide(const u32 *s_codes, const u32 *s_inval, u32 k, int mode, u32 bucket_bits,
                                                      u32 (&bk)[KP_ITEMS], const u32 t) {
  const u64 A  = ((u64)s_codes[t] << 32) | (u64)s_codes[t + 1];
  const u32 m  = (bucket_bits + 1) / 2, z0 = k - m;
  const u32 q  = z0 >> 4, r = z0 & 15u;
  const u64 H  = ((u64)s_codes[t + q] << 32) | (u64)s_codes[t + q + 1];
  const u64 L  = (q + 2 <= 4) ? ((u64)s_codes[t + q + 2] << 32) : 0ull;
  const u64 Z  = r ? ((H << (2 * r)) | (L >> (64 - 2 * r))) : H;
  const u64 RC = revcomp64(Z, 0);
  const u64 mmask = (1ull << (2 * m)) - 1ull;
  const u32 odd = 2 * m - bucket_bits;
#pragma unroll
  for (int j = 0; j < KP_ITEMS; j++) {
    const u32 ft = (u32)(((j == 0) ? A : (A << (2 * j))) >> (64 - bucket_bits));
    const u32 rt = (u32)((RC >> (2 * j)) & mmask) >> odd;
    bk[j] = (mode == 1) ? ft : (mode == 2) ? rt : (ft < rt ? ft : rt);
  }
  u128 X = ((u128)s_inval[t] << 112) | ((u128)s_inval[t + 1] << 96) | ((u128)s_inval[t + 2] << 80) |
           ((u128)s_inval[t + 3] << 64) | ((u128)s_inval[t + 4] << 48);
  u32 c = 1;
  while (2 * c <= k) { X |= X << c; c *= 2; }
  if (c < k) X |= X << (k - c);
  return __brev((u32)(~X >> 112) & 0xFFFFu) >> 16;
}

__device__ __forceinline__ u32 kp_thread_kmers(const u32 *s_codes, const u32 *s_inval, u32 k, int mode,
                                               K128 (&keys)[KP_ITEMS]) {
  const u32 t = threadIdx.x;
  const u128 A = ((u128)s_codes[t] << 96) | ((u128)s_codes[t + 1] << 64) | ((u128)s_codes[t + 2] << 32) |
                 (u128)s_codes[t + 3];
  const u128 B = (u128)s_codes[t + 4] << 96;
  const u128 I = ((u128)s_inval[t] << 112) | ((u128)s_inval[t + 1] << 96) | ((u128)s_inval[t + 2] << 80) |
                 ((u128)s_inval[t + 3] << 64) | ((u128)s_inval[t + 4] << 48);
  const u32 key_shift = 128 - 2 * k;
  const u32 top_shift = 2 * k - 2;
  u32 vmask = 0;
  u128 r = 0;
#pragma unroll
  for (int j = 0; j < KP_ITEMS; j++) {
    const u128 top = (j == 0) ? A : ((A << (2 * j)) | (B >> (128 - 2 * j)));
    const u128 f   = top >> key_shift;
    if (j == 0) {
      const u128 c = f ^ (((u128)0xAAAAAAAAAAAAAAAAull << 64) | (u128)0xAAAAAAAAAAAAAAAAull);
      u64 lo = __brevll((u64)(c >> 64)), hi = __brevll((u64)c);
      lo = ((lo >> 1) & 0x5555555555555555ull) | ((lo & 0x5555555555555555ull) << 1);
      hi = ((hi >> 1) & 0x5555555555555555ull) | ((hi & 0x5555555555555555ull) << 1);
      r = (((u128)hi << 64) | (u128)lo) >> key_shift;
    } else {
      r = (r >> 2) | ((u128)(((u64)f & 3ull) ^ 2ull) << top_shift);
    }
    const bool ok = (((I << j) >> (128 - k)) == (u128)0);
    u128 key;
    if      (mode == 1) key = f;
    else if (mode == 2) key = r;
    else                key = (f < r) ? f : r;
    keys[j] = KeyOps<K128>::mk(key);
    vmask |= (ok ? 1u : 0u) << j;
  }
  return vmask;
}

template <typename K>
__device__ __forceinline__ u32 kp_suffix_filter(const K (&keys)[KP_ITEMS], u32 vmask, u64 sfx_mask, u64 sfx_test) {
  if (sfx_mask == 0) return vmask;
#pragma unroll
  for (int j = 0; j < KP_ITEMS; j++)
    if ((KeyOps<K>::low64(keys[j]) & sfx_mask) != sfx_test) vmask &= ~(1u << j);
  return vmask;
}

__device__ __forceinline__ void kp_tile_range(u64 num_tiles, u64 &t_begin, u64 &t_end, u32 vwg = blockIdx.x, u32 vgrid = gridDim.x) {
  const u64 per = (num_tiles + vgrid - 1) / vgrid;
  t_begin = (u64)vwg * per;
  t_end   = t_begin + per;
  if (t_begin > num_tiles) t_begin = num_tiles;
  if (t_end   > num_tiles) t_end   = num_tiles;
}

template <typename K>
__global__ __launch_bounds__(KP_BLOCK)
void kmer_hist_kernel(const uint8_t *__restrict__ bases, u64 n, u32 k, int mode, u32 bucket_bits,
                      u64 num_tiles, u64 *__restrict__ block_hist, u64 *__restrict__ bucket_counts, u64 sfx_mask, u64 sfx_test) {
  __shared__ u32 s_codes[KP_WORDS];
  __shared__ u32 s_inval[KP_WORDS];
  __shared__ u32 s_hist[KP_MAX_BUCKETS];

  const u32  nb = 1u << bucket_bits;
  const u32  bucket_shift = 2 * k - bucket_bits;
  const bool aligned = ((reinterpret_cast<uintptr_t>(bases) & 15) == 0);

  for (u32 b = threadIdx.x; b < nb; b += KP_BLOCK) s_hist[b] = 0;
  __syncthreads();

  u64 t_begin, t_end;
  kp_tile_range(num_tiles, t_begin, t_end);
  u32 my_count = 0;

  for (u64 tile = t_begin; tile < t_end; tile++) {
    kp_stage_tile(bases, n, tile * KP_TILE, aligned, s_codes, s_inval);
    __syncthreads();
    if (sizeof(K) == 8 && nb > 1 && 2 * k >= bucket_bits && sfx_mask == 0) {
      u32 bk[KP_ITEMS];
      const u32 vmask = kp_thread_buckets(s_codes, s_inval, k, mode, bucket_bits, bk);
#pragma unroll
      for (int j = 0; j < KP_ITEMS; j++)
        if ((vmask >> j) & 1u) atomicAdd(&s_hist[bk[j]], 1u);
    } else {
      K keys[KP_ITEMS];
      const u32 vmask = kp_suffix_filter(keys, kp_thread_kmers(s_codes, s_inval, k, mode, keys), sfx_mask, sfx_test);
      if (nb == 1) {
        my_count += __popc(vmask);
      } else {
#pragma unroll
        for (int j = 0; j < KP_ITEMS; j++)
          if ((vmask >> j) & 1u) atomicAdd(&s_hist[KeyOps<K>::bucket(keys[j], bucket_shift)], 1u);
      }
    }
    __syncthreads();
  }
  if (nb == 1) atomicAdd(&s_hist[0], my_count);
  __syncthreads();

  for (u32 b = threadIdx.x; b < nb; b += KP_BLOCK) {
    const u64 v = s_hist[b];
    block_hist[(u64)blockIdx.x * nb + b] = v;
    if (v) atomicAdd(&bucket_counts[b], v);
  }
}

constexpr int KH_NV = 4, KH_FINE_BITS = 15;

__host__ __device__ constexpr u32 hpc_table_size(int hb) { u32 t = 4; for (int i = 1; i < hb; i++) t *= 3; return t; }
template <int HB>
__device__ __forceinline__ u32 hpc_dense_rank(u32 x) {
  u32 prev = (x >> (2 * HB - 2)) & 3u, r = prev;
#pragma unroll
  for (int i = 1; i < HB; i++) {
    const u32 c = (x >> (2 * (HB - 1 - i))) & 3u;
    r = r * 3u + (c - (c > prev ? 1u : 0u));
    prev = c;
  }
  return r;
}

template <int HB, int KC = 0>
__global__ __launch_bounds__(KP_BLOCK * KH_NV)
void kmer_hist_fine_kernel(const uint8_t *__restrict__ bases, u64 n, u32 k_arg, int mode_arg, u64 num_tiles, u32 vgrid,
                           u64 *__restrict__ block_hist, u64 *__restrict__ bucket_counts, u64 *__restrict__ fine_hist,
                           u32 fbits = 6 ,
                           u32 nvp = KH_NV ) {
  const u32 k = KC ? (u32)KC : k_arg;
  const int mode = KC ? 0 : mode_arg;
  constexpr u32 TABLE = HB ? hpc_table_size(HB) : (1u << KH_FINE_BITS);
  constexpr u32 NBK = HB ? (1u << (2 * (HB - 5))) : 64u;
  constexpr u32 IDX_BITS = HB ? 2u * HB : (u32)KH_FINE_BITS;
  extern __shared__ __attribute__((aligned(16))) u32 kh_fine[];
  __shared__ u32 s_codes[2][KH_NV][KP_WORDS];
  __shared__ u32 s_inval[2][KH_NV][KP_WORDS];
  __shared__ u32 s_prev[HB ? NBK : 256u];
  __shared__ unsigned short s_r5[HB ? 4096 : 1];
  __shared__ unsigned short s_rb[HB ? NBK : 1];
  const u32 tid = threadIdx.x, v = tid >> 8, t = tid & 255u;
  if constexpr (HB > 0) {
    for (u32 i = tid; i < 4096u; i += KP_BLOCK * KH_NV) s_r5[i] = (unsigned short)hpc_digit(i);
    if (tid < NBK) s_rb[tid] = (unsigned short)(hpc_dense_rank<HB - 5>(tid) * 243u);
  }
  const bool aligned = ((reinterpret_cast<uintptr_t>(bases) & 15) == 0);
  for (u32 i = tid; i < TABLE; i += KP_BLOCK * KH_NV) kh_fine[i] = 0;
  if (tid < (HB ? NBK : 256u)) s_prev[tid] = 0;

  const u64 per = (num_tiles + vgrid - 1) / vgrid;
  for (u32 vv = 0; vv < nvp; vv++) {
    const u64 vwg = (u64)blockIdx.x * nvp + vv;
    u64 t_begin = vwg * per, t_end = t_begin + per;
    if (t_begin > num_tiles) t_begin = num_tiles;
    if (t_end > num_tiles) t_end = num_tiles;
    if (vwg >= vgrid) t_begin = t_end = num_tiles;

    uint4 cur = make_uint4(0, 0, 0, 0), halo = make_uint4(0, 0, 0, 0);
    auto fetch = [&](u64 tile) {
      if (tile >= t_end) return;
      cur = load16(bases, tile * KP_TILE + (u64)t * 16, n, aligned);
      if (t < 4) halo = load16(bases, tile * KP_TILE + (u64)KP_TILE + (u64)t * 16, n, aligned);
    };
    fetch(t_begin + v);
    __syncthreads();
    const u64 rounds = (t_end - t_begin + KH_NV - 1) / KH_NV;
    for (u64 it = 0; it < rounds; it++) {
      const u64 tile = t_begin + it * KH_NV + v;
      const u32 buf = (u32)it & 1u;
      const bool active = tile < t_end;
      if (active) {
        u32 c, iv;
        encode16(cur, c, iv);
        s_codes[buf][v][t] = c; s_inval[buf][v][t] = iv;
        if (t < 4) { encode16(halo, c, iv); s_codes[buf][v][KP_BLOCK + t] = c; s_inval[buf][v][KP_BLOCK + t] = iv; }
      }
      __syncthreads();
      fetch(tile + KH_NV);
      if (active) {
        u32 bk[KP_ITEMS];
        const u32 vmask = (k > 32) ? kp_thread_buckets_wide(s_codes[buf][v], s_inval[buf][v], k, mode, IDX_BITS, bk, t)
                                   : kp_thread_buckets(s_codes[buf][v], s_inval[buf][v], k, mode, IDX_BITS, bk, t);
#pragma unroll
        for (int j = 0; j < KP_ITEMS; j++)
          if ((vmask >> j) & 1u) {
            if constexpr (HB > 0) { const u32 r = (u32)s_rb[bk[j] >> 10] + (u32)s_r5[bk[j] & 0xFFFu]; atomicAdd(&kh_fine[r < TABLE ? r : TABLE - 1u], 1u); }
            else atomicAdd(&kh_fine[bk[j]], 1u);
          }
      }
    }
    __syncthreads();
    {
      constexpr u32 TPB = (u32)(KP_BLOCK * KH_NV) / NBK;
      const u32 f = tid / TPB, l = tid % TPB;
      u32 sum = 0;
      (void)f; (void)l; (void)sum;
      if constexpr (HB > 0) {
        constexpr int BB = HB - 5;
        bool ok = true;
#pragma unroll
        for (int i = 1; i < BB; i++) ok = ok && (((f >> (2 * (BB - 1 - i))) & 3u) != ((f >> (2 * (BB - i))) & 3u));
        if (ok) { const u32 r0 = hpc_dense_rank<BB>(f) * 243u; for (u32 i = l; i < 243u; i += TPB) sum += kh_fine[r0 + i]; }
      }
      if constexpr (HB > 0) {
#pragma unroll
        for (u32 o = TPB / 2; o > 0; o >>= 1) sum += __shfl_xor(sum, o);
        if (l == 0) {
          const u32 c = sum - s_prev[f];
          s_prev[f] = sum;
          if (vwg < vgrid) block_hist[vwg * NBK + f] = c;
          if (c) atomicAdd(&bucket_counts[f], (u64)c);
        }
      } else if (fbits == 6) {
        for (u32 i = l; i < (1u << (KH_FINE_BITS - 6)); i += TPB) sum += kh_fine[(f << (KH_FINE_BITS - 6)) + i];
#pragma unroll
        for (u32 o = TPB / 2; o > 0; o >>= 1) sum += __shfl_xor(sum, o);
        if (l == 0) {
          const u32 c = sum - s_prev[f];
          s_prev[f] = sum;
          if (vwg < vgrid) block_hist[vwg * NBK + f] = c;
          if (c) atomicAdd(&bucket_counts[f], (u64)c);
        }
      } else {
        const u32 tpb = (u32)(KP_BLOCK * KH_NV) >> fbits, fr = tid / tpb, lr = tid % tpb, per_bucket = 1u << (KH_FINE_BITS - fbits);
        u32 rs = 0;
        for (u32 i = lr; i < per_bucket; i += tpb) rs += kh_fine[(fr << (KH_FINE_BITS - fbits)) + i];
        for (u32 o = tpb / 2; o > 0; o >>= 1) rs += __shfl_xor(rs, o);
        if (lr == 0) {
          const u32 c = rs - s_prev[fr];
          s_prev[fr] = rs;
          if (vwg < vgrid) block_hist[(vwg << fbits) + fr] = c;
          if (c) atomicAdd(&bucket_counts[fr], (u64)c);
        }
      }
    }
  }
  __syncthreads();
  for (u32 i = tid; i < TABLE; i += KP_BLOCK * KH_NV) {
    const u32 c = kh_fine[i];
    if (c) atomicAdd(&fine_hist[i], (u64)c);
  }
}

__global__ __launch_bounds__(256)
void kmer_scan_kernel(u64 *__restrict__ block_hist, u32 grid, u32 nb, const u64 *__restrict__ bucket_starts) {
  __shared__ u64 s_tmp[256 / 64 + 1];
  const u32 b = blockIdx.x;
  u64 carry = bucket_starts[b];
  for (u32 base = 0; base < grid; base += 256 * 8) {
    u64 v[8], sum = 0;
#pragma unroll
    for (int q = 0; q < 8; q++) {
      const u32 g = base + threadIdx.x * 8 + q;
      v[q] = (g < grid) ? block_hist[(u64)g * nb + b] : 0ull;
      sum += v[q];
    }
    u64 tot;
    u64 run = carry + block_excl_scan<256, u64>(sum, s_tmp, &tot);
#pragma unroll
    for (int q = 0; q < 8; q++) {
      const u32 g = base + threadIdx.x * 8 + q;
      if (g < grid) block_hist[(u64)g * nb + b] = run;
      run += v[q];
    }
    carry += tot;
  }
}

typedef __attribute__((address_space(1))) u32     kp_gu32;
typedef __attribute__((address_space(1))) uint8_t kp_gu8;
typedef __attribute__((address_space(1))) u64     kp_gu64;
typedef u32 kp_u32x3 __attribute__((ext_vector_type(3)));
typedef __attribute__((address_space(1))) __attribute__((aligned(4))) kp_u32x3 kp_gu32x3;
__device__ __forceinline__ void kp_gstore32(u64 addr, u32 v)     { *reinterpret_cast<kp_gu32 *>(addr) = v; }
__device__ __forceinline__ void kp_gstore8(u64 addr, uint8_t v)  { *reinterpret_cast<kp_gu8 *>(addr) = v; }
__device__ __forceinline__ void kp_gstore64(u64 addr, u64 v)     { *reinterpret_cast<kp_gu64 *>(addr) = v; }
__device__ __forceinline__ void kp_gstore96(u64 addr, u32 a, u32 b, u32 c) { kp_u32x3 v; v.x = a; v.y = b; v.z = c; *reinterpret_cast<kp_gu32x3 *>(addr) = v; }

template <typename K, int MAXB, bool SOA = false, int KC = 0, int BB = 6>
__global__ __launch_bounds__(KP_BLOCK, (sizeof(K) == 16) ? 2 : 4)
void kmer_partition_kernel(const uint8_t *__restrict__ bases, u64 n, u32 k_arg, int mode_arg, u32 bucket_bits_arg,
                           u64 num_tiles, const u64 *__restrict__ block_base, K *__restrict__ out, u64 sfx_mask_arg, u64 sfx_test,
                           const u64 *__restrict__ soa_starts = nullptr, const u64 *__restrict__ soa_counts = nullptr,
                           u32 vgrid = 0 ) {
  const u32 k = KC ? (u32)KC : k_arg;
  const int mode = KC ? 0 : mode_arg;
  const u32 bucket_bits = KC ? (u32)BB : bucket_bits_arg;
  const u64 sfx_mask = KC ? 0ull : sfx_mask_arg;
  static_assert(KC == 0 || MAXB >= (1 << BB), "the buckets of a constant-k form fit its tables");
  extern __shared__ __attribute__((aligned(16))) unsigned char kp_dyn_smem[];
  K *s_keys = reinterpret_cast<K *>(kp_dyn_smem);
  __shared__ u64 s_cursor[MAXB];
  __shared__ u32 s_cnt[MAXB];
  __shared__ u32 s_base[MAXB];
  __shared__ u32 s_codes[KP_WORDS];
  __shared__ u32 s_inval[KP_WORDS];
  __shared__ u32 s_tmp[KP_BLOCK / 64 + 1];

  const u32  nb = 1u << bucket_bits;
  const u32  bucket_shift = 2 * k - bucket_bits;
  const bool aligned = ((reinterpret_cast<uintptr_t>(bases) & 15) == 0);
  const u32  tid = threadIdx.x;

  __shared__ u64 s_fstart[SOA ? MAXB : 1], s_fhi[SOA ? MAXB : 1];
  constexpr bool OB = MAXB <= 64;
  __shared__ u64 s_ob[OB ? MAXB : 1], s_ob_hi[SOA ? MAXB : 1];
  static_assert(!SOA || OB, "the 5-byte layout is a 64-file layout");
  if constexpr (SOA) {
    for (u32 b = tid; b < nb; b += KP_BLOCK) {
      s_fstart[b] = soa_starts[b];
      if constexpr (sizeof(K) == 8) s_fhi[b] = 8ull * soa_starts[b] + 4ull * soa_counts[b];
      else                          s_fhi[b] = soa_counts[b];
    }
  }

  const u32 nvirt = vgrid ? vgrid : gridDim.x;
  for (u32 vwg = blockIdx.x; vwg < nvirt; vwg += gridDim.x) {
  __syncthreads();
  for (u32 b = tid; b < nb; b += KP_BLOCK) s_cursor[b] = block_base[(u64)vwg * nb + b];
  u64 t_begin, t_end;
  kp_tile_range(num_tiles, t_begin, t_end, vwg, nvirt);

  uint4 nx = make_uint4(0, 0, 0, 0), nx_halo = make_uint4(0, 0, 0, 0);
  auto prefetch = [&](u64 tile) __attribute__((always_inline)) {
    if (tile >= t_end) return;
    nx = load16(bases, tile * KP_TILE + (u64)tid * 16, n, aligned);
    if (tid < 4) nx_halo = load16(bases, tile * KP_TILE + (u64)KP_TILE + (u64)tid * 16, n, aligned);
  };
  prefetch(t_begin);
  for (u64 tile = t_begin; tile < t_end; tile++) {
    for (u32 b = tid; b < nb; b += KP_BLOCK) s_cnt[b] = 0;
    {
      u32 c, iv;
      encode16(nx, c, iv);
      s_codes[tid] = c; s_inval[tid] = iv;
      if (tid < 4) { encode16(nx_halo, c, iv); s_codes[KP_BLOCK + tid] = c; s_inval[KP_BLOCK + tid] = iv; }
    }
    prefetch(tile + 1);
    __syncthreads();

    K keys[KP_ITEMS];
    const u32 vmask = kp_suffix_filter(keys, kp_thread_kmers(s_codes, s_inval, k, mode, keys), sfx_mask, sfx_test);
    u32 total = 0;

    if (nb == 1) {
      const u32 c = __popc(vmask);
      const u32 base = block_excl_scan<KP_BLOCK, u32>(c, s_tmp, &total);
      u32 o = base;
#pragma unroll
      for (int j = 0; j < KP_ITEMS; j++)
        if ((vmask >> j) & 1u) s_keys[o++] = keys[j];
      if (tid == 0) { s_base[0] = 0; s_cnt[0] = total; if constexpr (OB) s_ob[0] = reinterpret_cast<u64>(out) + (u64)sizeof(K) * s_cursor[0]; }
      __syncthreads();
    } else {
      u32 ranks[KP_ITEMS];
#pragma unroll
      for (int j = 0; j < KP_ITEMS; j++) {
        ranks[j] = 0;
        if ((vmask >> j) & 1u) ranks[j] = atomicAdd(&s_cnt[KeyOps<K>::bucket(keys[j], bucket_shift)], 1u);
      }
      __syncthreads();
      u32 v[4], sum = 0;
#pragma unroll
      for (int q = 0; q < 4; q++) {
        const u32 b = tid * 4 + q;
        v[q] = (b < nb) ? s_cnt[b] : 0u;
        sum += v[q];
      }
      u32 run = block_excl_scan<KP_BLOCK, u32>(sum, s_tmp, &total);
#pragma unroll
      for (int q = 0; q < 4; q++) {
        const u32 b = tid * 4 + q;
        if (b < nb) {
          s_base[b] = run;
          if constexpr (SOA && sizeof(K) == 8) {
            const u64 rel0 = s_cursor[b] - s_fstart[b] - (u64)run;
            s_ob[b]    = reinterpret_cast<u64>(out) + 8ull * s_fstart[b] + 4ull * rel0;
            s_ob_hi[b] = reinterpret_cast<u64>(out) + s_fhi[b] + rel0;
          } else if constexpr (SOA) {
            const u64 rel0 = s_cursor[b] - s_fstart[b] - (u64)run;
            s_ob[b] = (reinterpret_cast<u64>(out) + 16ull * s_fstart[b] + (s_fhi[b] ? 12ull : 16ull) * rel0) | (s_fhi[b] ? 1ull : 0ull);
          } else if constexpr (OB) {
            s_ob[b] = reinterpret_cast<u64>(out) + (u64)sizeof(K) * (s_cursor[b] - (u64)run);
          }
        }
        run += v[q];
      }
      __syncthreads();
#pragma unroll
      for (int j = 0; j < KP_ITEMS; j++)
        if ((vmask >> j) & 1u) s_keys[s_base[KeyOps<K>::bucket(keys[j], bucket_shift)] + ranks[j]] = keys[j];
      __syncthreads();
    }

    for (u32 i = tid; i < total; i += KP_BLOCK) {
      const K   key = s_keys[i];
      const u32 b   = (nb == 1) ? 0u : KeyOps<K>::bucket(key, bucket_shift);
      if constexpr (SOA && sizeof(K) == 8) {
        kp_gstore32(s_ob[b] + 4ull * i, (u32)KeyOps<K>::low64(key));
        kp_gstore8(s_ob_hi[b] + (u64)i, (uint8_t)(KeyOps<K>::low64(key) >> 32));
      }
      else if constexpr (SOA) {
        const u64 ob = s_ob[b];
        const bool f96 = (ob & 1ull) != 0;
        const u64 addr = (ob & ~1ull) + (u64)(f96 ? 12u : 16u) * i;
        kp_gstore96(addr, (u32)key.lo, (u32)(key.lo >> 32), (u32)key.hi);
        if (!f96) kp_gstore32(addr + 12ull, (u32)(key.hi >> 32));
      }
      else if constexpr (OB) {
        if constexpr (sizeof(K) == 8) kp_gstore64(s_ob[b] + 8ull * i, (u64)KeyOps<K>::low64(key));
        else *reinterpret_cast<K *>(s_ob[b] + (u64)sizeof(K) * i) = key;
      }
      else out[s_cursor[b] + (u64)(i - s_base[b])] = key;
    }
    __syncthreads();
    for (u32 b = tid; b < nb; b += KP_BLOCK) s_cursor[b] += s_cnt[b];
    __syncthreads();
  }
  }
}

static int kmer_const_k(uint32_t k, int mode, bool on) {
  if (!on || mode != 0) return 0;
  return (k == 21 || k == 31 || k == 51) ? (int)k : 0;
}

constexpr uint32_t KP_VGRID = 16384, KP_PHYS = 2048;
static uint32_t kp_vgrid_max(uint32_t bucket_bits) {
  static const uint32_t env = [] { const char *e = getenv("MGC_PART_VGRID"); return (e && *e) ? (uint32_t)atoi(e) : 0u; }();
  if (bucket_bits > 8) return KP_PHYS;
  return (env >= 256 && env <= KP_VGRID) ? env : KP_PHYS;
}
uint32_t kp_grid_size(uint64_t n_bases, uint32_t bucket_bits) {
  const uint64_t num_tiles = (n_bases + KP_TILE - 1) / KP_TILE;
  const uint64_t vmax = kp_vgrid_max(bucket_bits);
  uint64_t g = num_tiles < vmax ? num_tiles : vmax;
  return (uint32_t)(g ? g : 1);
}

size_t kp_workspace_bytes(uint32_t bucket_bits) {
  return (size_t)(bucket_bits > 8 ? KP_PHYS : KP_VGRID) * ((size_t)1 << bucket_bits) * sizeof(uint64_t);
}

hipError_t launch_kmer_histogram(const uint8_t *d_bases, uint64_t n_bases, uint32_t k, int mode,
                                 uint32_t bucket_bits, uint64_t *d_bucket_counts, void *d_ws, hipStream_t st,
                                 uint64_t sfx_mask, uint64_t sfx_test) {
  const uint32_t nb = 1u << bucket_bits;
  MGC_CHECK(hipMemsetAsync(d_bucket_counts, 0, sizeof(uint64_t) * nb, st));
  if (n_bases == 0) return hipSuccess;
  const uint64_t num_tiles = (n_bases + KP_TILE - 1) / KP_TILE;
  const uint32_t grid = kp_grid_size(n_bases, bucket_bits);
  if (k <= 32)
    hipLaunchKernelGGL(kmer_hist_kernel<u64>, dim3(grid), dim3(KP_BLOCK), 0, st,
                       d_bases, (u64)n_bases, k, mode, bucket_bits, (u64)num_tiles,
                       reinterpret_cast<u64 *>(d_ws), reinterpret_cast<u64 *>(d_bucket_counts), (u64)sfx_mask, (u64)sfx_test);
  else
    hipLaunchKernelGGL(kmer_hist_kernel<K128>, dim3(grid), dim3(KP_BLOCK), 0, st,
                       d_bases, (u64)n_bases, k, mode, bucket_bits, (u64)num_tiles,
                       reinterpret_cast<u64 *>(d_ws), reinterpret_cast<u64 *>(d_bucket_counts), (u64)sfx_mask, (u64)sfx_test);
  return hipGetLastError();
}

bool kmer_histogram_fine_ok(uint32_t k, uint32_t bucket_bits, uint64_t sfx_mask, const Switches &sw) {
  return sw.fine_hist && k <= 64 && 2 * k >= (uint32_t)KH_FINE_BITS + 2 && bucket_bits == 6 && sfx_mask == 0;
}
bool kmer_histogram_fine_bits_ok(uint32_t k, uint32_t bucket_bits) { return k <= 64 && 2 * k >= (uint32_t)KH_FINE_BITS + 2 && bucket_bits >= 6 && bucket_bits <= 8; }

hipError_t launch_kmer_histogram_fine(const uint8_t *d_bases, uint64_t n_bases, uint32_t k, int mode, uint64_t *d_bucket_counts,
                                      uint64_t *d_fine_hist, void *d_ws, hipStream_t st, bool const_k, uint32_t bucket_bits) {
  if (bucket_bits < 6 || bucket_bits > 8) return hipErrorInvalidValue;
  MGC_CHECK(hipMemsetAsync(d_bucket_counts, 0, sizeof(uint64_t) << bucket_bits, st));
  MGC_CHECK(hipMemsetAsync(d_fine_hist, 0, sizeof(uint64_t) << KH_FINE_BITS, st));
  if (n_bases == 0) return hipSuccess;
  const uint64_t num_tiles = (n_bases + KP_TILE - 1) / KP_TILE;
  const uint32_t vgrid = kp_grid_size(n_bases, bucket_bits);
  const uint32_t nvp = std::max<uint32_t>((uint32_t)KH_NV, (vgrid + 511u) / 512u);
  static bool attr_done = false;
  if (!attr_done) {
    (void)hipFuncSetAttribute(reinterpret_cast<const void *>(&kmer_hist_fine_kernel<0>), hipFuncAttributeMaxDynamicSharedMemorySize,
                              (int)(sizeof(u32) << KH_FINE_BITS));
    (void)hipFuncSetAttribute(reinterpret_cast<const void *>(&kmer_hist_fine_kernel<0, 21>), hipFuncAttributeMaxDynamicSharedMemorySize,
                              (int)(sizeof(u32) << KH_FINE_BITS));
    (void)hipFuncSetAttribute(reinterpret_cast<const void *>(&kmer_hist_fine_kernel<0, 31>), hipFuncAttributeMaxDynamicSharedMemorySize,
                              (int)(sizeof(u32) << KH_FINE_BITS));
    (void)hipFuncSetAttribute(reinterpret_cast<const void *>(&kmer_hist_fine_kernel<0, 51>), hipFuncAttributeMaxDynamicSharedMemorySize,
                              (int)(sizeof(u32) << KH_FINE_BITS));
    attr_done = true;
  }
#define MGC_KH_LAUNCH(KC_)                                                                                                             \
  hipLaunchKernelGGL((kmer_hist_fine_kernel<0, KC_>), dim3((vgrid + nvp - 1) / nvp), dim3(KP_BLOCK * KH_NV), sizeof(u32) << KH_FINE_BITS, st, \
                     d_bases, (u64)n_bases, k, mode, (u64)num_tiles, vgrid, reinterpret_cast<u64 *>(d_ws),                             \
                     reinterpret_cast<u64 *>(d_bucket_counts), reinterpret_cast<u64 *>(d_fine_hist), bucket_bits, nvp)
  const int kc = kmer_const_k(k, mode, const_k);
  if (kc == 21) MGC_KH_LAUNCH(21); else if (kc == 31) MGC_KH_LAUNCH(31); else if (kc == 51) MGC_KH_LAUNCH(51); else MGC_KH_LAUNCH(0);
#undef MGC_KH_LAUNCH
  return hipGetLastError();
}

bool kmer_histogram_hpc_ok(uint32_t k, uint32_t bucket_bits, uint64_t sfx_mask, const Switches &sw) {
  return sw.hpc_msd && (bucket_bits == 6 || bucket_bits == 8) && k <= 64 && 2 * k >= bucket_bits + 10 + 2 && sfx_mask == 0;
}
uint32_t kmer_histogram_hpc_entries(uint32_t bucket_bits) { return hpc_table_size((int)(bucket_bits / 2 + 5)); }

hipError_t launch_kmer_histogram_hpc(const uint8_t *d_bases, uint64_t n_bases, uint32_t k, int mode, uint32_t bucket_bits,
                                     uint64_t *d_bucket_counts, uint64_t *d_fine_hist, void *d_ws, hipStream_t st, bool const_k) {
  if (bucket_bits != 6 && bucket_bits != 8) return hipErrorInvalidValue;
  const uint32_t entries = kmer_histogram_hpc_entries(bucket_bits);
  MGC_CHECK(hipMemsetAsync(d_bucket_counts, 0, sizeof(uint64_t) << bucket_bits, st));
  MGC_CHECK(hipMemsetAsync(d_fine_hist, 0, sizeof(uint64_t) * entries, st));
  if (n_bases == 0) return hipSuccess;
  const uint64_t num_tiles = (n_bases + KP_TILE - 1) / KP_TILE;
  const uint32_t vgrid = kp_grid_size(n_bases, bucket_bits);
  const uint32_t nvp = std::max<uint32_t>((uint32_t)KH_NV, (vgrid + 511u) / 512u);
  static bool attr_done = false;
  if (!attr_done) {
    (void)hipFuncSetAttribute(reinterpret_cast<const void *>(&kmer_hist_fine_kernel<8>), hipFuncAttributeMaxDynamicSharedMemorySize,
                              (int)(sizeof(u32) * hpc_table_size(8)));
    (void)hipFuncSetAttribute(reinterpret_cast<const void *>(&kmer_hist_fine_kernel<9>), hipFuncAttributeMaxDynamicSharedMemorySize,
                              (int)(sizeof(u32) * hpc_table_size(9)));
    (void)hipFuncSetAttribute(reinterpret_cast<const void *>(&kmer_hist_fine_kernel<8, 31>), hipFuncAttributeMaxDynamicSharedMemorySize,
                              (int)(sizeof(u32) * hpc_table_size(8)));
    (void)hipFuncSetAttribute(reinterpret_cast<const void *>(&kmer_hist_fine_kernel<9, 31>), hipFuncAttributeMaxDynamicSharedMemorySize,
                              (int)(sizeof(u32) * hpc_table_size(9)));
    attr_done = true;
  }
  const bool k31 = kmer_const_k(k, mode, const_k) == 31;
  if (k31 && bucket_bits == 6)
    hipLaunchKernelGGL((kmer_hist_fine_kernel<8, 31>), dim3((vgrid + nvp - 1) / nvp), dim3(KP_BLOCK * KH_NV), sizeof(u32) * entries, st,
                       d_bases, (u64)n_bases, k, mode, (u64)num_tiles, vgrid, reinterpret_cast<u64 *>(d_ws),
                       reinterpret_cast<u64 *>(d_bucket_counts), reinterpret_cast<u64 *>(d_fine_hist), 6u, nvp);
  else if (k31)
    hipLaunchKernelGGL((kmer_hist_fine_kernel<9, 31>), dim3((vgrid + nvp - 1) / nvp), dim3(KP_BLOCK * KH_NV), sizeof(u32) * entries, st,
                       d_bases, (u64)n_bases, k, mode, (u64)num_tiles, vgrid, reinterpret_cast<u64 *>(d_ws),
                       reinterpret_cast<u64 *>(d_bucket_counts), reinterpret_cast<u64 *>(d_fine_hist), 6u, nvp);
  else if (bucket_bits == 6)
    hipLaunchKernelGGL(kmer_hist_fine_kernel<8>, dim3((vgrid + nvp - 1) / nvp), dim3(KP_BLOCK * KH_NV), sizeof(u32) * entries, st,
                       d_bases, (u64)n_bases, k, mode, (u64)num_tiles, vgrid, reinterpret_cast<u64 *>(d_ws),
                       reinterpret_cast<u64 *>(d_bucket_counts), reinterpret_cast<u64 *>(d_fine_hist), 6u, nvp);
  else
    hipLaunchKernelGGL(kmer_hist_fine_kernel<9>, dim3((vgrid + nvp - 1) / nvp), dim3(KP_BLOCK * KH_NV), sizeof(u32) * entries, st,
                       d_bases, (u64)n_bases, k, mode, (u64)num_tiles, vgrid, reinterpret_cast<u64 *>(d_ws),
                       reinterpret_cast<u64 *>(d_bucket_counts), reinterpret_cast<u64 *>(d_fine_hist), 6u, nvp);
  return hipGetLastError();
}

hipError_t launch_kmer_partition(const uint8_t *d_bases, uint64_t n_bases, uint32_t k, int mode,
                                 uint32_t bucket_bits, const uint64_t *d_bucket_starts, void *d_keys,
                                 void *d_ws, hipStream_t st, uint64_t sfx_mask, uint64_t sfx_test, const uint64_t *d_soa_counts, bool const_k) {
  if (n_bases == 0) return hipSuccess;
  const uint32_t nb = 1u << bucket_bits;
  const uint64_t num_tiles = (n_bases + KP_TILE - 1) / KP_TILE;
  const uint32_t rows = kp_grid_size(n_bases, bucket_bits);
  const uint32_t grid = rows < KP_PHYS ? rows : KP_PHYS;
  hipLaunchKernelGGL(kmer_scan_kernel, dim3(nb), dim3(256), 0, st,
                     reinterpret_cast<u64 *>(d_ws), rows, nb, reinterpret_cast<const u64 *>(d_bucket_starts));
  MGC_CHECK(hipGetLastError());
  static bool attr_done = false;
  if (!attr_done) {
    (void)hipFuncSetAttribute(reinterpret_cast<const void *>(&kmer_partition_kernel<K128, 64>),
                              hipFuncAttributeMaxDynamicSharedMemorySize, (int)(KP_TILE * sizeof(K128)));
    (void)hipFuncSetAttribute(reinterpret_cast<const void *>(&kmer_partition_kernel<K128, KP_MAX_BUCKETS>),
                              hipFuncAttributeMaxDynamicSharedMemorySize, (int)(KP_TILE * sizeof(K128)));
    (void)hipFuncSetAttribute(reinterpret_cast<const void *>(&kmer_partition_kernel<K128, 64, false, 51>),
                              hipFuncAttributeMaxDynamicSharedMemorySize, (int)(KP_TILE * sizeof(K128)));
    attr_done = true;
  }
#define MGC_KP_LAUNCH(K_, MAXB_)                                                                                   \
  hipLaunchKernelGGL((kmer_partition_kernel<K_, MAXB_>), dim3(grid), dim3(KP_BLOCK), KP_TILE * sizeof(K_), st,      \
                     d_bases, (u64)n_bases, k, mode, bucket_bits, (u64)num_tiles,                                  \
                     reinterpret_cast<const u64 *>(d_ws), reinterpret_cast<K_ *>(d_keys), (u64)sfx_mask, (u64)sfx_test, (const u64 *)nullptr, (const u64 *)nullptr, rows)
  if (d_soa_counts && k > 32) {
    if (!(k <= 51 && nb == 64 && sfx_mask == 0)) return hipErrorInvalidValue;
    static bool a96 = false;
    if (!a96) {
      (void)hipFuncSetAttribute(reinterpret_cast<const void *>(&kmer_partition_kernel<K128, 64, true>),
                                hipFuncAttributeMaxDynamicSharedMemorySize, (int)(KP_TILE * sizeof(K128)));
      (void)hipFuncSetAttribute(reinterpret_cast<const void *>(&kmer_partition_kernel<K128, 64, true, 51>),
                                hipFuncAttributeMaxDynamicSharedMemorySize, (int)(KP_TILE * sizeof(K128)));
      a96 = true;
    }
    if (kmer_const_k(k, mode, const_k) == 51)
      hipLaunchKernelGGL((kmer_partition_kernel<K128, 64, true, 51>), dim3(grid), dim3(KP_BLOCK), KP_TILE * sizeof(K128), st, d_bases, (u64)n_bases, k, mode,
                         bucket_bits, (u64)num_tiles, reinterpret_cast<const u64 *>(d_ws), reinterpret_cast<K128 *>(d_keys), (u64)0, (u64)0,
                         reinterpret_cast<const u64 *>(d_bucket_starts), reinterpret_cast<const u64 *>(d_soa_counts), rows);
    else
      hipLaunchKernelGGL((kmer_partition_kernel<K128, 64, true>), dim3(grid), dim3(KP_BLOCK), KP_TILE * sizeof(K128), st, d_bases, (u64)n_bases, k, mode,
                         bucket_bits, (u64)num_tiles, reinterpret_cast<const u64 *>(d_ws), reinterpret_cast<K128 *>(d_keys), (u64)0, (u64)0,
                         reinterpret_cast<const u64 *>(d_bucket_starts), reinterpret_cast<const u64 *>(d_soa_counts), rows);
    return hipGetLastError();
  }
  if (d_soa_counts) {
    if (!(k <= 32 && nb == 64 && sfx_mask == 0)) return hipErrorInvalidValue;
    if (kmer_const_k(k, mode, const_k) == 21)
      hipLaunchKernelGGL((kmer_partition_kernel<u64, 64, true, 21>), dim3(grid), dim3(KP_BLOCK), KP_TILE * sizeof(u64), st, d_bases, (u64)n_bases, k, mode,
                         bucket_bits, (u64)num_tiles, reinterpret_cast<const u64 *>(d_ws), reinterpret_cast<u64 *>(d_keys), (u64)0, (u64)0,
                         reinterpret_cast<const u64 *>(d_bucket_starts), reinterpret_cast<const u64 *>(d_soa_counts), rows);
    else
      hipLaunchKernelGGL((kmer_partition_kernel<u64, 64, true>), dim3(grid), dim3(KP_BLOCK), KP_TILE * sizeof(u64), st, d_bases, (u64)n_bases, k, mode,
                         bucket_bits, (u64)num_tiles, reinterpret_cast<const u64 *>(d_ws), reinterpret_cast<u64 *>(d_keys), (u64)0, (u64)0,
                         reinterpret_cast<const u64 *>(d_bucket_starts), reinterpret_cast<const u64 *>(d_soa_counts), rows);
    return hipGetLastError();
  }
#define MGC_KPC_LAUNCH(K_, KC_)                                                                                    \
  hipLaunchKernelGGL((kmer_partition_kernel<K_, 64, false, KC_>), dim3(grid), dim3(KP_BLOCK), KP_TILE * sizeof(K_), st, \
                     d_bases, (u64)n_bases, k, mode, bucket_bits, (u64)num_tiles,                                  \
                     reinterpret_cast<const u64 *>(d_ws), reinterpret_cast<K_ *>(d_keys), (u64)0, (u64)0, (const u64 *)nullptr, (const u64 *)nullptr, rows)
  const int kc = (nb == 64 && sfx_mask == 0) ? kmer_const_k(k, mode, const_k) : 0;
  if (nb == 256 && sfx_mask == 0 && kmer_const_k(k, mode, const_k) == 31)
    hipLaunchKernelGGL((kmer_partition_kernel<u64, 256, false, 31, 8>), dim3(grid), dim3(KP_BLOCK), KP_TILE * sizeof(u64), st,
                       d_bases, (u64)n_bases, k, mode, bucket_bits, (u64)num_tiles, reinterpret_cast<const u64 *>(d_ws), reinterpret_cast<u64 *>(d_keys), (u64)0, (u64)0, (const u64 *)nullptr, (const u64 *)nullptr, rows);
  else if (kc == 21) MGC_KPC_LAUNCH(u64, 21);
  else if (kc == 31) MGC_KPC_LAUNCH(u64, 31);
  else if (kc == 51) MGC_KPC_LAUNCH(K128, 51);
  else if (k <= 32) { if (nb <= 64) MGC_KP_LAUNCH(u64, 64); else MGC_KP_LAUNCH(u64, KP_MAX_BUCKETS); }
  else              { if (nb <= 64) MGC_KP_LAUNCH(K128, 64); else MGC_KP_LAUNCH(K128, KP_MAX_BUCKETS); }
#undef MGC_KPC_LAUNCH
#undef MGC_KP_LAUNCH
  return hipGetLastError();
}



hipError_t warm_kmer() { hipFuncAttributes a; return hipFuncGetAttributes(&a, reinterpret_cast<const void *>(&kmer_scan_kernel)); }

}
```

### meryl_amd/csrc/mgc_session.hpp

```cpp
#pragma once

#include "../../include/meryl_gpu_count.h"
#include "mgc_clock.hpp"
#include "mgc_device.h"

#include <cstdarg>
#include <cstdio>
#include <cstring>
#include <mutex>
#include <string>
#include <thread>
#include <vector>

namespace mgc {
std::string &thread_last_error();
bool effective_geometry(mgc_count_config *c);

inline void set_err(std::string *dst, const char *fmt, ...) {
  char buf[512];
  va_list ap;
  va_start(ap, fmt);
  vsnprintf(buf, sizeof(buf), fmt, ap);
  va_end(ap);
  if (dst) {
    static std::mutex mu;
    std::lock_guard<std::mutex> g(mu);
    *dst = buf;
  }
  thread_last_error() = buf;
}

struct DBuf {
  void *p = nullptr; size_t cap = 0;
  hipError_t ensure(size_t bytes) {
    if (bytes < 256) bytes = 256;
    if (cap >= bytes) return hipSuccess;
    if (p) { (void)hipFree(p); p = nullptr; cap = 0; }
    hipError_t e = hipMalloc(&p, bytes);
    if (e == hipSuccess) cap = bytes;
    return e;
  }
  void release() { if (p) (void)hipFree(p); p = nullptr; cap = 0; }
  template <typename T> T *as() const { return reinterpret_cast<T *>(p); }
};
}

#define HIP_TRY(s, expr)                                                                         \
  do {                                                                                           \
    hipError_t e__ = (expr);                                                                     \
    if (e__ != hipSuccess) {                                                                     \
      mgc::set_err((s) ? &(s)->err : nullptr, "%s:%d: %s -> %s", __FILE__, __LINE__, #expr,      \
                   hipGetErrorString(e__));                                                      \
      return (e__ == hipErrorOutOfMemory) ? MGC_ENOMEM : MGC_EHIP;                               \
    }                                                                                            \
  } while (0)

struct mgc_session {
  mgc_count_config cfg;
  int              device = -1;
  hipStream_t      stream = nullptr;
  uint64_t         sfx_mask = 0, sfx_test = 0;
  mgc::Switches    sw;
  static constexpr int HUGE_EXTRA = 3;
  hipStream_t      stream_h[HUGE_EXTRA] = {nullptr, nullptr, nullptr};
  hipStream_t      stream2 = nullptr;
  hipEvent_t       ev_fork = nullptr, ev_join = nullptr;
  uint64_t        *h_stats = nullptr;
  size_t           h_stats_cap = 0;
  std::string      err;

  const uint8_t    *d_bases = nullptr;
  uint64_t          n_bases = 0;
  bool              borrowed = false;

  bool      counted = false;
  uint64_t  n_instances = 0, n_distinct = 0;
  uint64_t  file_instances[MGC_NUM_FILES];
  void     *d_unique = nullptr;
  uint32_t *d_counts = nullptr;
  uint64_t *d_block_start = nullptr;
  uint32_t  key_words = 1;

  struct Buf { void *p = nullptr; size_t cap = 0; };
  enum { B_PART_WS, B_META, B_X, B_Y, B_SORT_WS, B_RLE_WS, B_UNIQUE, B_COUNTS, B_BLOCKS, B_HPC, B_HPC_WS,
         B_SUBSTART, B_GROUPS, B_GSCAN, B_CNT_TMP, B_LARGE, B_NONEMPTY, B_STAGE0, B_STAGE1, B_TEXT_IN0, B_TEXT_IN1, B_TEXT_WS,
         B_TEXT_STATE, B_RK, B_RC, B_R2K, B_R2C, B_MERGE_WS, B_SORT_HDRS, B_FINE, B_NARROW_WS, B_Y2, B_Y3, B_Y4, B_HWS0, B_HWS1, B_HWS2, B_HWS3, B_NUM };
  Buf buf[B_NUM];
  double tr_alloc = 0;
  uint64_t tr_alloc_bytes = 0;
  hipError_t ensure(int which, size_t bytes) {
    Buf &b = buf[which];
    if (bytes < 256) bytes = 256;
    if (b.cap >= bytes) return hipSuccess;
    const double t0 = mgc::now_s();
    if (b.p) { (void)hipFree(b.p); b.p = nullptr; b.cap = 0; }
    hipError_t e = hipMalloc(&b.p, bytes);
    if (e == hipSuccess) b.cap = bytes;
    tr_alloc += mgc::now_s() - t0;
    tr_alloc_bytes += bytes;
    return e;
  }
  void free_arena() { for (auto &b : buf) { if (b.p) (void)hipFree(b.p); b.p = nullptr; b.cap = 0; } }
  std::vector<void *> garbage;
  hipError_t ensure_preserve(int which, size_t bytes, size_t keep, hipStream_t on) {
    Buf &b = buf[which];
    if (b.cap >= bytes) return hipSuccess;
    struct Tm { double *acc; double t0; Tm(double *a) : acc(a), t0(mgc::now_s()) {} ~Tm() { *acc += mgc::now_s() - t0; } } tm_(&tr_grow);
    size_t want = b.cap * 4;
    const size_t full = batch_limit ? (size_t)batch_limit + 4 * PIN_CHUNK : 0;
    if (full && want > full && full >= bytes) want = full;
    if (want < bytes) want = bytes;
    void *np = nullptr;
    hipError_t e = hipMalloc(&np, want);
    if (e != hipSuccess && want > bytes) { want = bytes; e = hipMalloc(&np, want); }
    if (e != hipSuccess) return e;
    if (b.p && keep) e = hipMemcpyAsync(np, b.p, keep, hipMemcpyDeviceToDevice, on);
    if (e == hipSuccess) e = hipStreamSynchronize(on);
    if (b.p) garbage.push_back(b.p);
    b.p = np; b.cap = want;
    return e;
  }
  void free_garbage() { for (void *p : garbage) (void)hipFree(p); garbage.clear(); }

  static constexpr size_t TEXT_CHUNK = 32u << 20;
  static constexpr size_t PIN_CHUNK  = 32u << 20;
  hipStream_t st_in = nullptr;
  bool        state_ready = false;
  int         fill = 0;
  uint64_t    fill_len = 0;
  bool        len_inexact = false;
  bool        input_seen = false;
  bool        text_open = false, text_cut_in_file = false;
  int         text_format = 0;
  char       *text_pinned[2] = {nullptr, nullptr};
  hipEvent_t  text_ev[2] = {nullptr, nullptr};
  hipStream_t st_up = nullptr;
  hipEvent_t  up_ev[2] = {nullptr, nullptr};
  bool        text_ev_used[2] = {false, false};
  uint32_t    text_next = 0;
  static constexpr int TEXT_RING_MAX = 64;
  char       *text_ring[TEXT_RING_MAX] = {nullptr};
  char       *pin[2] = {nullptr, nullptr};
  size_t      pin_len = 0;
  int         pin_cur = 0;
  hipEvent_t  pin_ev[2] = {nullptr, nullptr};
  bool        pin_used[2] = {false, false};

  uint64_t    batch_limit = 0;
  uint64_t    no_cut_below = 0;
  bool        have_r = false;
  struct mgc_runs *runs = nullptr;
  bool        ooc = false;
  uint64_t    result_budget = 0;
  uint64_t    total_bases = 0, total_instances = 0;
  uint64_t    total_file_instances[MGC_NUM_FILES];
  uint32_t    n_batches = 0;
  double      merge_ms = 0;
  std::thread worker;
  double      tr_memcpy = 0, tr_flush = 0, tr_cut = 0, tr_join = 0, tr_grow = 0;
  bool        worker_active = false;
  int         worker_rc = MGC_OK;

  std::thread prep_thread;
  bool        prep_active = false;
  void join_prepare() { if (prep_active) { prep_thread.join(); prep_active = false; } }

  bool        profiling = false;
  mgc_profile prof;

  void free_result() {
    d_unique = nullptr; d_counts = nullptr; d_block_start = nullptr;
    counted = false;
  }
};

namespace mgc {
struct CountInput {
  void           *keys = nullptr;
  const uint64_t *counts = nullptr;
  uint32_t        bucket_bits = MGC_NUM_FILES_BITS;
  const uint64_t *fine = nullptr;
  void           *out_keys = nullptr;
  uint32_t       *out_counts = nullptr;
  uint64_t        out_cap = 0;
};
int count_device(mgc_session *s, const CountInput &in = CountInput());

int text_submit(mgc_session *s, const char *pinned_src, size_t piece);
void text_drain(mgc_session *s);
int text_rollback(mgc_session *s);
}
```

Measured before the change: 11.73 billion distinct k-mers/s.

## Cache 2-bit packed bases from histogram pass for reuse in partition pass

The histogram kernels now write the 2-bit encoded codes and invalid-base masks for each 16-base word into a packed device buffer. The partition kernel then reads this packed form instead of re-reading and re-encoding the raw ASCII bases. This cuts the partition pass's base reads to about 6 bytes per 16 bases instead of 16, and skips its re-encode. In exchange it adds extra writes in the histogram pass, a new allocation gated by a free-memory check, and a templated PK path that launches through a new dispatch helper.

```diff
diff --git a/meryl_amd/build.py b/meryl_amd/build.py
--- a/meryl_amd/build.py
+++ b/meryl_amd/build.py
@@ -9,7 +9,7 @@
 SOURCES = ["mgc_kmer.hip", "mgc_sort.hip", "mgc_scan.hip", "mgc_finish.hip", "mgc_misc.hip", "mgc_parse.hip",
            "mgc_encode.hip", "mgc_decode.hip", "mgc_merge.hip", "mgc_merge_many.hip", "mgc_lookup.hip", "mgc_filter.hip", "mgc_import.hip", "mgc_analyze.hip", "mgc_value_hist.hip",
            "mgc_api.cpp", "mgc_textfile.cpp", "mgc_import.cpp", "mgc_analyze.cpp", "mgc_count.cpp", "mgc_stream.cpp", "mgc_eval.cpp", "mgc_runs.cpp", "mgc_node.cpp", "meryl_db.cpp", "meryl_seq.cpp"]
-HEADERS = ["mgc_device.h", "mgc_common.hpp", "mdb_layout.h", "mdb_statistics.hpp", "mgc_session.hpp", "mgc_clock.hpp", "mgc_chunk_ring.hpp", "mgc_bgzf.hpp", "mgc_runs.hpp", "mgc_lookup_dev.hpp", "mgc_import_dev.hpp", "mgc_analyze_dev.hpp", "mgc_label.hpp", "mgc_selector.hpp", "mgc_value.hpp", "mgc_route.hpp",
+HEADERS = ["mgc_device.h", "mgc_common.hpp", "mgc_bases.hpp", "mdb_layout.h", "mdb_statistics.hpp", "mgc_session.hpp", "mgc_clock.hpp", "mgc_chunk_ring.hpp", "mgc_bgzf.hpp", "mgc_runs.hpp", "mgc_lookup_dev.hpp", "mgc_import_dev.hpp", "mgc_analyze_dev.hpp", "mgc_label.hpp", "mgc_selector.hpp", "mgc_value.hpp", "mgc_route.hpp",
            os.path.join("..", "..", "include", "meryl_gpu_count.h"),
            os.path.join("..", "..", "include", "meryl_db.h"), os.path.join("..", "..", "include", "meryl_seq.h"),
            os.path.join("..", "..", "include", "meryl_lookup.h"), os.path.join("..", "..", "include", "meryl_import.h"),
diff --git a/meryl_amd/csrc/mgc_api.cpp b/meryl_amd/csrc/mgc_api.cpp
--- a/meryl_amd/csrc/mgc_api.cpp
+++ b/meryl_amd/csrc/mgc_api.cpp
@@ -26,7 +26,7 @@
   auto on1 = [](const char *n) { const char *e = getenv(n); return e && e[0] == '1'; };
   auto num = [](const char *n, uint64_t d) { const char *e = getenv(n); return (e && *e) ? strtoull(e, nullptr, 10) : d; };
   sw.fine_hist = !off("MGC_FINE_HIST"); sw.hpc_msd = !off("MGC_HPC_MSD"); sw.hpc_digits = !off("MGC_HPC_DIGITS");
-  sw.const_k = !off("MGC_KMER_CONST_K"); sw.narrow = !off("MGC_NARROW"); sw.wide_msd = !off("MGC_WIDE_MSD");
+  sw.const_k = !off("MGC_KMER_CONST_K"); sw.packed_bases = !off("MGC_PACKED_BASES"); sw.narrow = !off("MGC_NARROW"); sw.wide_msd = !off("MGC_WIDE_MSD");
   sw.group_pipe = !off("MGC_GROUP_PIPE"); sw.soa5 = !off("MGC_SOA5"); sw.k96 = !off("MGC_K96"); sw.finish = !off("MGC_FINISH");
   sw.nolist = on1("MGC_FINISH_NOLIST");
   sw.finish_trace = getenv("MGC_FINISH_TRACE") != nullptr; sw.group_dbg = getenv("MGC_GROUP_DBG") != nullptr; sw.hash_dbg = getenv("MGC_HASH_DBG") != nullptr;
diff --git a/meryl_amd/csrc/mgc_bases.hpp b/meryl_amd/csrc/mgc_bases.hpp
--- /dev/null
+++ b/meryl_amd/csrc/mgc_bases.hpp
@@ -0,0 +1,40 @@
+#pragma once
+#include <cstdint>
+
+#if defined(__HIPCC__) || defined(__CUDACC__)
+#define MGC_BASES_FN __host__ __device__ __forceinline__
+#else
+#define MGC_BASES_FN inline
+#endif
+
+namespace mgc {
+
+MGC_BASES_FN uint32_t code_bytes4(uint32_t w) { return (w >> 1) & 0x03030303u; }
+
+MGC_BASES_FN uint32_t enc4_codes(uint32_t cb) { return (cb * 0x40100401u) >> 24; }
+MGC_BASES_FN uint32_t enc4(uint32_t w) { return enc4_codes(code_bytes4(w)); }
+
+MGC_BASES_FN uint32_t select_bytes4(uint32_t table, uint32_t sel) {
+#if defined(__HIP_DEVICE_COMPILE__)
+  return __builtin_amdgcn_perm(table, table, sel);
+#else
+  uint32_t r = 0;
+  for (int i = 0; i < 4; i++) r |= ((table >> (8u * ((sel >> (8 * i)) & 3u))) & 0xFFu) << (8 * i);
+  return r;
+#endif
+}
+
+MGC_BASES_FN uint32_t inv4_codes(uint32_t w, uint32_t cb) {
+  const uint32_t x  = (w & 0xDFDFDFDFu) ^ select_bytes4(0x47544341u, cb);
+  const uint32_t nz = (((x & 0x7F7F7F7Fu) + 0x7F7F7F7Fu) | x) & 0x80808080u;
+  return (((nz >> 7) * 0x08040201u) >> 24) & 0xFu;
+}
+MGC_BASES_FN uint32_t inv4(uint32_t w) { return inv4_codes(w, code_bytes4(w)); }
+
+MGC_BASES_FN void encode16(uint32_t x, uint32_t y, uint32_t z, uint32_t w, uint32_t &codes, uint32_t &inval) {
+  const uint32_t cx = code_bytes4(x), cy = code_bytes4(y), cz = code_bytes4(z), cw = code_bytes4(w);
+  codes = (enc4_codes(cx) << 24) | (enc4_codes(cy) << 16) | (enc4_codes(cz) << 8) | enc4_codes(cw);
+  inval = (inv4_codes(x, cx) << 12) | (inv4_codes(y, cy) << 8) | (inv4_codes(z, cz) << 4) | inv4_codes(w, cw);
+}
+
+}
diff --git a/meryl_amd/csrc/mgc_count.cpp b/meryl_amd/csrc/mgc_count.cpp
--- a/meryl_amd/csrc/mgc_count.cpp
+++ b/meryl_amd/csrc/mgc_count.cpp
@@ -262,6 +262,7 @@
   uint64_t *d_counts64 = nullptr, *d_starts = nullptr;
   std::vector<uint64_t> h_meta;
   const uint64_t *d_fine = nullptr, *d_fine_hpc = nullptr;
+  void *d_packed = nullptr;
   mgc::SortPlan full{};
   bool use_finish;
   unsigned char *X = nullptr, *Y = nullptr;
@@ -341,20 +342,33 @@
   std::vector<uint64_t> h_counts(nb);
   const bool wide_msd_on = sw.wide_msd && !c.homopoly_compress;
   if (!in.keys) {
+    if (sw.packed_bases && n_bases) {
+      const size_t pb = mgc::kp_packed_bytes(n_bases);
+      bool room = s->buf[S::B_PACKED].cap >= pb;
+      if (!room) {
+        size_t free_b = 0, total_b = 0;
+        room = hipMemGetInfo(&free_b, &total_b) == hipSuccess &&
+               (double)free_b + (double)s->arena_bytes() >= (double)n_bases * (double)(2 + 14ull * kw) + (double)pb;
+      }
+      if (room) {
+        if (s->ensure(S::B_PACKED, pb) == hipSuccess) d_packed = s->buf[S::B_PACKED].p;
+        else (void)hipGetLastError();
+      }
+    }
     tm.begin(MGC_STAGE_HISTOGRAM);
     if (n_bases >= (1u << 22) && ((kw == 1 && 2 * k - bucket_bits <= 41) || wide_msd_on) && mgc::kmer_histogram_fine_ok(k, bucket_bits, s->sfx_mask, sw)) {
       HIP_TRY(s, s->ensure(S::B_FINE, sizeof(uint64_t) << 15));
       uint64_t *fine = reinterpret_cast<uint64_t *>(s->buf[S::B_FINE].p);
-      HIP_TRY(s, mgc::launch_kmer_histogram_fine(d_bases, n_bases, k, c.mode, d_counts64, fine, part_ws, st, sw.const_k));
+      HIP_TRY(s, mgc::launch_kmer_histogram_fine(d_bases, n_bases, k, c.mode, d_counts64, fine, part_ws, st, sw.const_k, 6, d_packed));
       d_fine = fine;
     } else if (c.homopoly_compress && n_bases >= (1u << 22) && (2 * k - bucket_bits) % 2 == 0 && 2 * k - bucket_bits >= 20 &&
                sw.hpc_digits && mgc::kmer_histogram_hpc_ok(k, bucket_bits, s->sfx_mask, sw)) {
       HIP_TRY(s, s->ensure(S::B_FINE, sizeof(uint64_t) * std::max<size_t>((size_t)1 << 15, mgc::kmer_histogram_hpc_entries(bucket_bits))));
       uint64_t *fine = reinterpret_cast<uint64_t *>(s->buf[S::B_FINE].p);
-      HIP_TRY(s, mgc::launch_kmer_histogram_hpc(d_bases, n_bases, k, c.mode, bucket_bits, d_counts64, fine, part_ws, st, sw.const_k));
+      HIP_TRY(s, mgc::launch_kmer_histogram_hpc(d_bases, n_bases, k, c.mode, bucket_bits, d_counts64, fine, part_ws, st, sw.const_k, d_packed));
       d_fine_hpc = fine;
     } else
-    HIP_TRY(s, mgc::launch_kmer_histogram(d_bases, n_bases, k, c.mode, bucket_bits, d_counts64, part_ws, st, s->sfx_mask, s->sfx_test));
+    HIP_TRY(s, mgc::launch_kmer_histogram(d_bases, n_bases, k, c.mode, bucket_bits, d_counts64, part_ws, st, s->sfx_mask, s->sfx_test, d_packed));
     tm.end(MGC_STAGE_HISTOGRAM);
     prof.stage_launches[MGC_STAGE_HISTOGRAM] = 1;
     HIP_TRY(s, hipMemcpyAsync(h_counts.data(), d_counts64, sizeof(uint64_t) * nb, hipMemcpyDeviceToHost, st));
@@ -407,10 +421,11 @@
   if (k96) HIP_TRY(s, hipMemcpyAsync(d_k96flags, h_meta.data() + nb, sizeof(uint64_t) * nb, hipMemcpyHostToDevice, st));
   tm.begin(MGC_STAGE_PARTITION);
   HIP_TRY(s, mgc::launch_kmer_partition(d_bases, n_bases, k, c.mode, bucket_bits, d_starts, (void *)X, part_ws, st,
-                                        s->sfx_mask, s->sfx_test, k96 ? d_k96flags : (soa ? d_counts64 : nullptr), sw.const_k));
+                                        s->sfx_mask, s->sfx_test, k96 ? d_k96flags : (soa ? d_counts64 : nullptr), sw.const_k, d_packed));
   tm.end(MGC_STAGE_PARTITION);
-  prof.hist_bytes = n_bases;
-  prof.partition_bytes = n_bases;
+  const uint64_t packed_b = d_packed ? mgc::kp_packed_bytes(n_bases) : 0;
+  prof.hist_bytes = n_bases + packed_b;
+  prof.partition_bytes = d_packed ? packed_b : n_bases;
   for (uint32_t b = 0; b < nb; b++) prof.partition_bytes += plan.files[b].size * (soa ? 5u : ((k96 && plan.files[b].k96) ? 12u : (uint64_t)kbytes));
   prof.stage_launches[MGC_STAGE_PARTITION] = 2;
   return MGC_OK;
diff --git a/meryl_amd/csrc/mgc_device.h b/meryl_amd/csrc/mgc_device.h
--- a/meryl_amd/csrc/mgc_device.h
+++ b/meryl_amd/csrc/mgc_device.h
@@ -13,6 +13,7 @@
   bool hpc_msd = true;
   bool hpc_digits = true;
   bool const_k = true;
+  bool packed_bases = true;
   bool narrow = true;
   bool wide_msd = true;
   bool soa5 = true;
@@ -44,24 +45,27 @@
 
 uint32_t kp_grid_size(uint64_t n_bases, uint32_t bucket_bits);
 size_t   kp_workspace_bytes(uint32_t bucket_bits);
+size_t   kp_packed_bytes(uint64_t n_bases);
 
 bool       kmer_histogram_fine_ok(uint32_t k, uint32_t bucket_bits, uint64_t sfx_mask, const Switches &sw);
 bool       kmer_histogram_hpc_ok(uint32_t k, uint32_t bucket_bits, uint64_t sfx_mask, const Switches &sw);
 uint32_t   kmer_histogram_hpc_entries(uint32_t bucket_bits);
 hipError_t launch_kmer_histogram_hpc(const uint8_t *d_bases, uint64_t n_bases, uint32_t k, int mode, uint32_t bucket_bits,
-                                     uint64_t *d_bucket_counts, uint64_t *d_fine_hist, void *d_ws, hipStream_t st, bool const_k = true );
+                                     uint64_t *d_bucket_counts, uint64_t *d_fine_hist, void *d_ws, hipStream_t st, bool const_k = true ,
+                                     void *d_packed = nullptr);
 hipError_t launch_kmer_histogram_fine(const uint8_t *d_bases, uint64_t n_bases, uint32_t k, int mode, uint64_t *d_bucket_counts,
                                       uint64_t *d_fine_hist, void *d_ws, hipStream_t st, bool const_k = true ,
-                                      uint32_t bucket_bits = 6 );
+                                      uint32_t bucket_bits = 6 ,
+                                      void *d_packed = nullptr);
 bool       kmer_histogram_fine_bits_ok(uint32_t k, uint32_t bucket_bits);
 hipError_t launch_kmer_histogram(const uint8_t *d_bases, uint64_t n_bases, uint32_t k, int mode,
                                  uint32_t bucket_bits, uint64_t *d_bucket_counts, void *d_ws, hipStream_t st,
-                                 uint64_t sfx_mask = 0, uint64_t sfx_test = 0);
+                                 uint64_t sfx_mask = 0, uint64_t sfx_test = 0, void *d_packed = nullptr);
 hipError_t launch_kmer_partition(const uint8_t *d_bases, uint64_t n_bases, uint32_t k, int mode,
                                  uint32_t bucket_bits, const uint64_t *d_bucket_starts, void *d_keys,
                                  void *d_ws, hipStream_t st, uint64_t sfx_mask = 0, uint64_t sfx_test = 0,
                                  const uint64_t *d_soa_counts = nullptr ,
-                                 bool const_k = true );
+                                 bool const_k = true , void *d_packed = nullptr);
 
 struct SortPlan {
   uint32_t radix_bits;
diff --git a/meryl_amd/csrc/mgc_kmer.hip b/meryl_amd/csrc/mgc_kmer.hip
--- a/meryl_amd/csrc/mgc_kmer.hip
+++ b/meryl_amd/csrc/mgc_kmer.hip
@@ -1,27 +1,12 @@
 #include "mgc_common.hpp"
+#include "mgc_bases.hpp"
 
 namespace mgc {
 
 
-__device__ __forceinline__ u32 enc4(u32 w) {
-  return (((w >> 1) & 0x03030303u) * 0x40100401u) >> 24;
-}
-__device__ __forceinline__ u32 zero_bytes(u32 x) {
-  return ~(((x & 0x7F7F7F7Fu) + 0x7F7F7F7Fu) | x | 0x7F7F7F7Fu);
-}
-__device__ __forceinline__ u32 inv4(u32 w) {
-  const u32 u = w & 0xDFDFDFDFu;
-  const u32 ok = zero_bytes(u ^ 0x41414141u) | zero_bytes(u ^ 0x43434343u) |
-                 zero_bytes(u ^ 0x47474747u) | zero_bytes(u ^ 0x54545454u);
-  const u32 g = ((~ok) & 0x80808080u) >> 7;
-  return ((g * 0x08040201u) >> 24) & 0xFu;
-}
-
-
-__device__ __forceinline__ void encode16(uint4 v, u32 &codes, u32 &inval) {
-  codes = (enc4(v.x) << 24) | (enc4(v.y) << 16) | (enc4(v.z) << 8) | enc4(v.w);
-  inval = (inv4(v.x) << 12) | (inv4(v.y) << 8) | (inv4(v.z) << 4) | inv4(v.w);
-}
+__device__ __forceinline__ void encode16(uint4 v, u32 &codes, u32 &inval) { encode16(v.x, v.y, v.z, v.w, codes, inval); }
+
+struct PackedBases { u32 *codes; unsigned short *inval; };
 
 __device__ __forceinline__ u64 revcomp64(u64 f, u32 key_shift ) {
   u64 x = __brevll(f ^ 0xAAAAAAAAAAAAAAAAull);
@@ -32,17 +17,20 @@
 constexpr int KP_WORDS = KP_TILE / 16 + 4;
 
 __device__ __forceinline__ void kp_stage_tile(const uint8_t *__restrict__ bases, u64 n, u64 tile0, bool aligned,
-                                              u32 *s_codes, u32 *s_inval) {
+                                              u32 *s_codes, u32 *s_inval, PackedBases pk, bool last) {
   const u32 t = threadIdx.x;
+  const u64 w0 = tile0 / 16;
   {
     u32 c, iv;
     encode16(load16(bases, tile0 + (u64)t * 16, n, aligned), c, iv);
     s_codes[t] = c; s_inval[t] = iv;
+    if (pk.codes) { pk.codes[w0 + t] = c; pk.inval[w0 + t] = (unsigned short)iv; }
   }
   if (t < 4) {
     u32 c, iv;
     encode16(load16(bases, tile0 + (u64)KP_TILE + (u64)t * 16, n, aligned), c, iv);
     s_codes[KP_BLOCK + t] = c; s_inval[KP_BLOCK + t] = iv;
+    if (pk.codes && last) { pk.codes[w0 + KP_BLOCK + t] = c; pk.inval[w0 + KP_BLOCK + t] = (unsigned short)iv; }
   }
 }
 
@@ -179,7 +167,8 @@
 template <typename K>
 __global__ __launch_bounds__(KP_BLOCK)
 void kmer_hist_kernel(const uint8_t *__restrict__ bases, u64 n, u32 k, int mode, u32 bucket_bits,
-                      u64 num_tiles, u64 *__restrict__ block_hist, u64 *__restrict__ bucket_counts, u64 sfx_mask, u64 sfx_test) {
+                      u64 num_tiles, u64 *__restrict__ block_hist, u64 *__restrict__ bucket_counts, u64 sfx_mask, u64 sfx_test,
+                      PackedBases pk) {
   __shared__ u32 s_codes[KP_WORDS];
   __shared__ u32 s_inval[KP_WORDS];
   __shared__ u32 s_hist[KP_MAX_BUCKETS];
@@ -196,7 +185,7 @@
   u32 my_count = 0;
 
   for (u64 tile = t_begin; tile < t_end; tile++) {
-    kp_stage_tile(bases, n, tile * KP_TILE, aligned, s_codes, s_inval);
+    kp_stage_tile(bases, n, tile * KP_TILE, aligned, s_codes, s_inval, pk, tile + 1 == num_tiles);
     __syncthreads();
     if (sizeof(K) == 8 && nb > 1 && 2 * k >= bucket_bits && sfx_mask == 0) {
       u32 bk[KP_ITEMS];
@@ -247,7 +236,8 @@
 void kmer_hist_fine_kernel(const uint8_t *__restrict__ bases, u64 n, u32 k_arg, int mode_arg, u64 num_tiles, u32 vgrid,
                            u64 *__restrict__ block_hist, u64 *__restrict__ bucket_counts, u64 *__restrict__ fine_hist,
                            u32 fbits = 6 ,
-                           u32 nvp = KH_NV ) {
+                           u32 nvp = KH_NV ,
+                           PackedBases pk = PackedBases{nullptr, nullptr} ) {
   const u32 k = KC ? (u32)KC : k_arg;
   const int mode = KC ? 0 : mode_arg;
   constexpr u32 TABLE = HB ? hpc_table_size(HB) : (1u << KH_FINE_BITS);
@@ -293,7 +283,12 @@
         u32 c, iv;
         encode16(cur, c, iv);
         s_codes[buf][v][t] = c; s_inval[buf][v][t] = iv;
-        if (t < 4) { encode16(halo, c, iv); s_codes[buf][v][KP_BLOCK + t] = c; s_inval[buf][v][KP_BLOCK + t] = iv; }
+        const u64 w0 = tile * (u64)KP_BLOCK;
+        if (pk.codes) { pk.codes[w0 + t] = c; pk.inval[w0 + t] = (unsigned short)iv; }
+        if (t < 4) {
+          encode16(halo, c, iv); s_codes[buf][v][KP_BLOCK + t] = c; s_inval[buf][v][KP_BLOCK + t] = iv;
+          if (pk.codes && tile + 1 == num_tiles) { pk.codes[w0 + KP_BLOCK + t] = c; pk.inval[w0 + KP_BLOCK + t] = (unsigned short)iv; }
+        }
       }
       __syncthreads();
       fetch(tile + KH_NV);
@@ -397,12 +392,13 @@
 __device__ __forceinline__ void kp_gstore64(u64 addr, u64 v)     { *reinterpret_cast<kp_gu64 *>(addr) = v; }
 __device__ __forceinline__ void kp_gstore96(u64 addr, u32 a, u32 b, u32 c) { kp_u32x3 v; v.x = a; v.y = b; v.z = c; *reinterpret_cast<kp_gu32x3 *>(addr) = v; }
 
-template <typename K, int MAXB, bool SOA = false, int KC = 0, int BB = 6>
+template <typename K, int MAXB, bool SOA = false, int KC = 0, int BB = 6, bool PK = false>
 __global__ __launch_bounds__(KP_BLOCK, (sizeof(K) == 16) ? 2 : 4)
 void kmer_partition_kernel(const uint8_t *__restrict__ bases, u64 n, u32 k_arg, int mode_arg, u32 bucket_bits_arg,
                            u64 num_tiles, const u64 *__restrict__ block_base, K *__restrict__ out, u64 sfx_mask_arg, u64 sfx_test,
                            const u64 *__restrict__ soa_starts = nullptr, const u64 *__restrict__ soa_counts = nullptr,
-                           u32 vgrid = 0 ) {
+                           u32 vgrid = 0 ,
+                           PackedBases pk = PackedBases{nullptr, nullptr}) {
   const u32 k = KC ? (u32)KC : k_arg;
   const int mode = KC ? 0 : mode_arg;
   const u32 bucket_bits = KC ? (u32)BB : bucket_bits_arg;
@@ -444,13 +440,22 @@
   uint4 nx = make_uint4(0, 0, 0, 0), nx_halo = make_uint4(0, 0, 0, 0);
   auto prefetch = [&](u64 tile) __attribute__((always_inline)) {
     if (tile >= t_end) return;
-    nx = load16(bases, tile * KP_TILE + (u64)tid * 16, n, aligned);
-    if (tid < 4) nx_halo = load16(bases, tile * KP_TILE + (u64)KP_TILE + (u64)tid * 16, n, aligned);
+    if constexpr (PK) {
+      const u64 w0 = tile * (u64)KP_BLOCK;
+      nx.x = pk.codes[w0 + tid]; nx.y = pk.inval[w0 + tid];
+      if (tid < 4) { nx_halo.x = pk.codes[w0 + KP_BLOCK + tid]; nx_halo.y = pk.inval[w0 + KP_BLOCK + tid]; }
+    } else {
+      nx = load16(bases, tile * KP_TILE + (u64)tid * 16, n, aligned);
+      if (tid < 4) nx_halo = load16(bases, tile * KP_TILE + (u64)KP_TILE + (u64)tid * 16, n, aligned);
+    }
   };
   prefetch(t_begin);
   for (u64 tile = t_begin; tile < t_end; tile++) {
     for (u32 b = tid; b < nb; b += KP_BLOCK) s_cnt[b] = 0;
-    {
+    if constexpr (PK) {
+      s_codes[tid] = nx.x; s_inval[tid] = nx.y;
+      if (tid < 4) { s_codes[KP_BLOCK + tid] = nx_halo.x; s_inval[KP_BLOCK + tid] = nx_halo.y; }
+    } else {
       u32 c, iv;
       encode16(nx, c, iv);
       s_codes[tid] = c; s_inval[tid] = iv;
@@ -562,9 +567,18 @@
   return (size_t)(bucket_bits > 8 ? KP_PHYS : KP_VGRID) * ((size_t)1 << bucket_bits) * sizeof(uint64_t);
 }
 
+static uint64_t kp_packed_words(uint64_t n_bases) { return (n_bases + KP_TILE - 1) / KP_TILE * (uint64_t)KP_BLOCK + 4; }
+size_t kp_packed_bytes(uint64_t n_bases) { return (size_t)(kp_packed_words(n_bases) * 6); }
+static PackedBases kp_packed(void *d_packed, uint64_t n_bases) {
+  if (!d_packed) return PackedBases{nullptr, nullptr};
+  u32 *codes = reinterpret_cast<u32 *>(d_packed);
+  return PackedBases{codes, reinterpret_cast<unsigned short *>(codes + kp_packed_words(n_bases))};
+}
+
 hipError_t launch_kmer_histogram(const uint8_t *d_bases, uint64_t n_bases, uint32_t k, int mode,
                                  uint32_t bucket_bits, uint64_t *d_bucket_counts, void *d_ws, hipStream_t st,
-                                 uint64_t sfx_mask, uint64_t sfx_test) {
+                                 uint64_t sfx_mask, uint64_t sfx_test, void *d_packed) {
+  const PackedBases pk = kp_packed(d_packed, n_bases);
   const uint32_t nb = 1u << bucket_bits;
   MGC_CHECK(hipMemsetAsync(d_bucket_counts, 0, sizeof(uint64_t) * nb, st));
   if (n_bases == 0) return hipSuccess;
@@ -573,11 +587,11 @@
   if (k <= 32)
     hipLaunchKernelGGL(kmer_hist_kernel<u64>, dim3(grid), dim3(KP_BLOCK), 0, st,
                        d_bases, (u64)n_bases, k, mode, bucket_bits, (u64)num_tiles,
-                       reinterpret_cast<u64 *>(d_ws), reinterpret_cast<u64 *>(d_bucket_counts), (u64)sfx_mask, (u64)sfx_test);
+                       reinterpret_cast<u64 *>(d_ws), reinterpret_cast<u64 *>(d_bucket_counts), (u64)sfx_mask, (u64)sfx_test, pk);
   else
     hipLaunchKernelGGL(kmer_hist_kernel<K128>, dim3(grid), dim3(KP_BLOCK), 0, st,
                        d_bases, (u64)n_bases, k, mode, bucket_bits, (u64)num_tiles,
-                       reinterpret_cast<u64 *>(d_ws), reinterpret_cast<u64 *>(d_bucket_counts), (u64)sfx_mask, (u64)sfx_test);
+                       reinterpret_cast<u64 *>(d_ws), reinterpret_cast<u64 *>(d_bucket_counts), (u64)sfx_mask, (u64)sfx_test, pk);
   return hipGetLastError();
 }
 
@@ -587,8 +601,10 @@
 bool kmer_histogram_fine_bits_ok(uint32_t k, uint32_t bucket_bits) { return k <= 64 && 2 * k >= (uint32_t)KH_FINE_BITS + 2 && bucket_bits >= 6 && bucket_bits <= 8; }
 
 hipError_t launch_kmer_histogram_fine(const uint8_t *d_bases, uint64_t n_bases, uint32_t k, int mode, uint64_t *d_bucket_counts,
-                                      uint64_t *d_fine_hist, void *d_ws, hipStream_t st, bool const_k, uint32_t bucket_bits) {
+                                      uint64_t *d_fine_hist, void *d_ws, hipStream_t st, bool const_k, uint32_t bucket_bits,
+                                      void *d_packed) {
   if (bucket_bits < 6 || bucket_bits > 8) return hipErrorInvalidValue;
+  const PackedBases pk = kp_packed(d_packed, n_bases);
   MGC_CHECK(hipMemsetAsync(d_bucket_counts, 0, sizeof(uint64_t) << bucket_bits, st));
   MGC_CHECK(hipMemsetAsync(d_fine_hist, 0, sizeof(uint64_t) << KH_FINE_BITS, st));
   if (n_bases == 0) return hipSuccess;
@@ -610,7 +626,7 @@
 #define MGC_KH_LAUNCH(KC_)                                                                                                             \
   hipLaunchKernelGGL((kmer_hist_fine_kernel<0, KC_>), dim3((vgrid + nvp - 1) / nvp), dim3(KP_BLOCK * KH_NV), sizeof(u32) << KH_FINE_BITS, st, \
                      d_bases, (u64)n_bases, k, mode, (u64)num_tiles, vgrid, reinterpret_cast<u64 *>(d_ws),                             \
-                     reinterpret_cast<u64 *>(d_bucket_counts), reinterpret_cast<u64 *>(d_fine_hist), bucket_bits, nvp)
+                     reinterpret_cast<u64 *>(d_bucket_counts), reinterpret_cast<u64 *>(d_fine_hist), bucket_bits, nvp, pk)
   const int kc = kmer_const_k(k, mode, const_k);
   if (kc == 21) MGC_KH_LAUNCH(21); else if (kc == 31) MGC_KH_LAUNCH(31); else if (kc == 51) MGC_KH_LAUNCH(51); else MGC_KH_LAUNCH(0);
 #undef MGC_KH_LAUNCH
@@ -623,8 +639,10 @@
 uint32_t kmer_histogram_hpc_entries(uint32_t bucket_bits) { return hpc_table_size((int)(bucket_bits / 2 + 5)); }
 
 hipError_t launch_kmer_histogram_hpc(const uint8_t *d_bases, uint64_t n_bases, uint32_t k, int mode, uint32_t bucket_bits,
-                                     uint64_t *d_bucket_counts, uint64_t *d_fine_hist, void *d_ws, hipStream_t st, bool const_k) {
+                                     uint64_t *d_bucket_counts, uint64_t *d_fine_hist, void *d_ws, hipStream_t st, bool const_k,
+                                     void *d_packed) {
   if (bucket_bits != 6 && bucket_bits != 8) return hipErrorInvalidValue;
+  const PackedBases pk = kp_packed(d_packed, n_bases);
   const uint32_t entries = kmer_histogram_hpc_entries(bucket_bits);
   MGC_CHECK(hipMemsetAsync(d_bucket_counts, 0, sizeof(uint64_t) << bucket_bits, st));
   MGC_CHECK(hipMemsetAsync(d_fine_hist, 0, sizeof(uint64_t) * entries, st));
@@ -648,25 +666,51 @@
   if (k31 && bucket_bits == 6)
     hipLaunchKernelGGL((kmer_hist_fine_kernel<8, 31>), dim3((vgrid + nvp - 1) / nvp), dim3(KP_BLOCK * KH_NV), sizeof(u32) * entries, st,
                        d_bases, (u64)n_bases, k, mode, (u64)num_tiles, vgrid, reinterpret_cast<u64 *>(d_ws),
-                       reinterpret_cast<u64 *>(d_bucket_counts), reinterpret_cast<u64 *>(d_fine_hist), 6u, nvp);
+                       reinterpret_cast<u64 *>(d_bucket_counts), reinterpret_cast<u64 *>(d_fine_hist), 6u, nvp, pk);
   else if (k31)
     hipLaunchKernelGGL((kmer_hist_fine_kernel<9, 31>), dim3((vgrid + nvp - 1) / nvp), dim3(KP_BLOCK * KH_NV), sizeof(u32) * entries, st,
                        d_bases, (u64)n_bases, k, mode, (u64)num_tiles, vgrid, reinterpret_cast<u64 *>(d_ws),
-                       reinterpret_cast<u64 *>(d_bucket_counts), reinterpret_cast<u64 *>(d_fine_hist), 6u, nvp);
+                       reinterpret_cast<u64 *>(d_bucket_counts), reinterpret_cast<u64 *>(d_fine_hist), 6u, nvp, pk);
   else if (bucket_bits == 6)
     hipLaunchKernelGGL(kmer_hist_fine_kernel<8>, dim3((vgrid + nvp - 1) / nvp), dim3(KP_BLOCK * KH_NV), sizeof(u32) * entries, st,
                        d_bases, (u64)n_bases, k, mode, (u64)num_tiles, vgrid, reinterpret_cast<u64 *>(d_ws),
-                       reinterpret_cast<u64 *>(d_bucket_counts), reinterpret_cast<u64 *>(d_fine_hist), 6u, nvp);
+                       reinterpret_cast<u64 *>(d_bucket_counts), reinterpret_cast<u64 *>(d_fine_hist), 6u, nvp, pk);
   else
     hipLaunchKernelGGL(kmer_hist_fine_kernel<9>, dim3((vgrid + nvp - 1) / nvp), dim3(KP_BLOCK * KH_NV), sizeof(u32) * entries, st,
                        d_bases, (u64)n_bases, k, mode, (u64)num_tiles, vgrid, reinterpret_cast<u64 *>(d_ws),
-                       reinterpret_cast<u64 *>(d_bucket_counts), reinterpret_cast<u64 *>(d_fine_hist), 6u, nvp);
+                       reinterpret_cast<u64 *>(d_bucket_counts), reinterpret_cast<u64 *>(d_fine_hist), 6u, nvp, pk);
   return hipGetLastError();
+}
+
+struct KpLaunch {
+  const uint8_t *d_bases; uint64_t n_bases; uint32_t k; int mode; uint32_t bucket_bits; uint64_t num_tiles;
+  void *d_ws, *d_keys; uint64_t sfx_mask, sfx_test; const u64 *soa_starts, *soa_counts; uint32_t rows, grid; hipStream_t st;
+  PackedBases pk;
+};
+template <typename K, int MAXB, bool SOA, int KC, int BB, bool PK>
+static void kp_launch_form(const KpLaunch &a) {
+  if constexpr (sizeof(K) == 16) {
+    static bool attr_done = false;
+    if (!attr_done) {
+      (void)hipFuncSetAttribute(reinterpret_cast<const void *>(&kmer_partition_kernel<K, MAXB, SOA, KC, BB, PK>),
+                                hipFuncAttributeMaxDynamicSharedMemorySize, (int)(KP_TILE * sizeof(K)));
+      attr_done = true;
+    }
+  }
+  hipLaunchKernelGGL((kmer_partition_kernel<K, MAXB, SOA, KC, BB, PK>), dim3(a.grid), dim3(KP_BLOCK), KP_TILE * sizeof(K), a.st,
+                     a.d_bases, (u64)a.n_bases, a.k, a.mode, a.bucket_bits, (u64)a.num_tiles, reinterpret_cast<const u64 *>(a.d_ws),
+                     reinterpret_cast<K *>(a.d_keys), (u64)a.sfx_mask, (u64)a.sfx_test, a.soa_starts, a.soa_counts, a.rows, a.pk);
+}
+template <typename K, int MAXB, bool SOA, int KC, int BB = 6>
+static void kp_launch(const KpLaunch &a) {
+  if (a.pk.codes) kp_launch_form<K, MAXB, SOA, KC, BB, true>(a);
+  else            kp_launch_form<K, MAXB, SOA, KC, BB, false>(a);
 }
 
 hipError_t launch_kmer_partition(const uint8_t *d_bases, uint64_t n_bases, uint32_t k, int mode,
                                  uint32_t bucket_bits, const uint64_t *d_bucket_starts, void *d_keys,
-                                 void *d_ws, hipStream_t st, uint64_t sfx_mask, uint64_t sfx_test, const uint64_t *d_soa_counts, bool const_k) {
+                                 void *d_ws, hipStream_t st, uint64_t sfx_mask, uint64_t sfx_test, const uint64_t *d_soa_counts, bool const_k,
+                                 void *d_packed) {
   if (n_bases == 0) return hipSuccess;
   const uint32_t nb = 1u << bucket_bits;
   const uint64_t num_tiles = (n_bases + KP_TILE - 1) / KP_TILE;
@@ -675,67 +719,23 @@
   hipLaunchKernelGGL(kmer_scan_kernel, dim3(nb), dim3(256), 0, st,
                      reinterpret_cast<u64 *>(d_ws), rows, nb, reinterpret_cast<const u64 *>(d_bucket_starts));
   MGC_CHECK(hipGetLastError());
-  static bool attr_done = false;
-  if (!attr_done) {
-    (void)hipFuncSetAttribute(reinterpret_cast<const void *>(&kmer_partition_kernel<K128, 64>),
-                              hipFuncAttributeMaxDynamicSharedMemorySize, (int)(KP_TILE * sizeof(K128)));
-    (void)hipFuncSetAttribute(reinterpret_cast<const void *>(&kmer_partition_kernel<K128, KP_MAX_BUCKETS>),
-                              hipFuncAttributeMaxDynamicSharedMemorySize, (int)(KP_TILE * sizeof(K128)));
-    (void)hipFuncSetAttribute(reinterpret_cast<const void *>(&kmer_partition_kernel<K128, 64, false, 51>),
-                              hipFuncAttributeMaxDynamicSharedMemorySize, (int)(KP_TILE * sizeof(K128)));
-    attr_done = true;
-  }
-#define MGC_KP_LAUNCH(K_, MAXB_)                                                                                   \
-  hipLaunchKernelGGL((kmer_partition_kernel<K_, MAXB_>), dim3(grid), dim3(KP_BLOCK), KP_TILE * sizeof(K_), st,      \
-                     d_bases, (u64)n_bases, k, mode, bucket_bits, (u64)num_tiles,                                  \
-                     reinterpret_cast<const u64 *>(d_ws), reinterpret_cast<K_ *>(d_keys), (u64)sfx_mask, (u64)sfx_test, (const u64 *)nullptr, (const u64 *)nullptr, rows)
-  if (d_soa_counts && k > 32) {
-    if (!(k <= 51 && nb == 64 && sfx_mask == 0)) return hipErrorInvalidValue;
-    static bool a96 = false;
-    if (!a96) {
-      (void)hipFuncSetAttribute(reinterpret_cast<const void *>(&kmer_partition_kernel<K128, 64, true>),
-                                hipFuncAttributeMaxDynamicSharedMemorySize, (int)(KP_TILE * sizeof(K128)));
-      (void)hipFuncSetAttribute(reinterpret_cast<const void *>(&kmer_partition_kernel<K128, 64, true, 51>),
-                                hipFuncAttributeMaxDynamicSharedMemorySize, (int)(KP_TILE * sizeof(K128)));
-      a96 = true;
-    }
-    if (kmer_const_k(k, mode, const_k) == 51)
-      hipLaunchKernelGGL((kmer_partition_kernel<K128, 64, true, 51>), dim3(grid), dim3(KP_BLOCK), KP_TILE * sizeof(K128), st, d_bases, (u64)n_bases, k, mode,
-                         bucket_bits, (u64)num_tiles, reinterpret_cast<const u64 *>(d_ws), reinterpret_cast<K128 *>(d_keys), (u64)0, (u64)0,
-                         reinterpret_cast<const u64 *>(d_bucket_starts), reinterpret_cast<const u64 *>(d_soa_counts), rows);
-    else
-      hipLaunchKernelGGL((kmer_partition_kernel<K128, 64, true>), dim3(grid), dim3(KP_BLOCK), KP_TILE * sizeof(K128), st, d_bases, (u64)n_bases, k, mode,
-                         bucket_bits, (u64)num_tiles, reinterpret_cast<const u64 *>(d_ws), reinterpret_cast<K128 *>(d_keys), (u64)0, (u64)0,
-                         reinterpret_cast<const u64 *>(d_bucket_starts), reinterpret_cast<const u64 *>(d_soa_counts), rows);
+  const KpLaunch a{d_bases, n_bases, k, mode, bucket_bits, num_tiles, d_ws, d_keys, sfx_mask, sfx_test, nullptr, nullptr, rows, grid, st,
+                   kp_packed(d_packed, n_bases)};
+  const int kck = (sfx_mask == 0) ? kmer_const_k(k, mode, const_k) : 0;
+  if (d_soa_counts) {
+    if (!(nb == 64 && sfx_mask == 0 && k <= 51)) return hipErrorInvalidValue;
+    KpLaunch s = a;
+    s.soa_starts = reinterpret_cast<const u64 *>(d_bucket_starts); s.soa_counts = reinterpret_cast<const u64 *>(d_soa_counts);
+    if (k > 32) { if (kck == 51) kp_launch<K128, 64, true, 51>(s); else kp_launch<K128, 64, true, 0>(s); }
+    else        { if (kck == 21) kp_launch<u64, 64, true, 21>(s);  else kp_launch<u64, 64, true, 0>(s); }
     return hipGetLastError();
   }
-  if (d_soa_counts) {
-    if (!(k <= 32 && nb == 64 && sfx_mask == 0)) return hipErrorInvalidValue;
-    if (kmer_const_k(k, mode, const_k) == 21)
-      hipLaunchKernelGGL((kmer_partition_kernel<u64, 64, true, 21>), dim3(grid), dim3(KP_BLOCK), KP_TILE * sizeof(u64), st, d_bases, (u64)n_bases, k, mode,
-                         bucket_bits, (u64)num_tiles, reinterpret_cast<const u64 *>(d_ws), reinterpret_cast<u64 *>(d_keys), (u64)0, (u64)0,
-                         reinterpret_cast<const u64 *>(d_bucket_starts), reinterpret_cast<const u64 *>(d_soa_counts), rows);
-    else
-      hipLaunchKernelGGL((kmer_partition_kernel<u64, 64, true>), dim3(grid), dim3(KP_BLOCK), KP_TILE * sizeof(u64), st, d_bases, (u64)n_bases, k, mode,
-                         bucket_bits, (u64)num_tiles, reinterpret_cast<const u64 *>(d_ws), reinterpret_cast<u64 *>(d_keys), (u64)0, (u64)0,
-                         reinterpret_cast<const u64 *>(d_bucket_starts), reinterpret_cast<const u64 *>(d_soa_counts), rows);
-    return hipGetLastError();
-  }
-#define MGC_KPC_LAUNCH(K_, KC_)                                                                                    \
-  hipLaunchKernelGGL((kmer_partition_kernel<K_, 64, false, KC_>), dim3(grid), dim3(KP_BLOCK), KP_TILE * sizeof(K_), st, \
-                     d_bases, (u64)n_bases, k, mode, bucket_bits, (u64)num_tiles,                                  \
-                     reinterpret_cast<const u64 *>(d_ws), reinterpret_cast<K_ *>(d_keys), (u64)0, (u64)0, (const u64 *)nullptr, (const u64 *)nullptr, rows)
-  const int kc = (nb == 64 && sfx_mask == 0) ? kmer_const_k(k, mode, const_k) : 0;
-  if (nb == 256 && sfx_mask == 0 && kmer_const_k(k, mode, const_k) == 31)
-    hipLaunchKernelGGL((kmer_partition_kernel<u64, 256, false, 31, 8>), dim3(grid), dim3(KP_BLOCK), KP_TILE * sizeof(u64), st,
-                       d_bases, (u64)n_bases, k, mode, bucket_bits, (u64)num_tiles, reinterpret_cast<const u64 *>(d_ws), reinterpret_cast<u64 *>(d_keys), (u64)0, (u64)0, (const u64 *)nullptr, (const u64 *)nullptr, rows);
-  else if (kc == 21) MGC_KPC_LAUNCH(u64, 21);
-  else if (kc == 31) MGC_KPC_LAUNCH(u64, 31);
-  else if (kc == 51) MGC_KPC_LAUNCH(K128, 51);
-  else if (k <= 32) { if (nb <= 64) MGC_KP_LAUNCH(u64, 64); else MGC_KP_LAUNCH(u64, KP_MAX_BUCKETS); }
-  else              { if (nb <= 64) MGC_KP_LAUNCH(K128, 64); else MGC_KP_LAUNCH(K128, KP_MAX_BUCKETS); }
-#undef MGC_KPC_LAUNCH
-#undef MGC_KP_LAUNCH
+  if (nb == 256 && kck == 31) kp_launch<u64, 256, false, 31, 8>(a);
+  else if (nb == 64 && kck == 21) kp_launch<u64, 64, false, 21>(a);
+  else if (nb == 64 && kck == 31) kp_launch<u64, 64, false, 31>(a);
+  else if (nb == 64 && kck == 51) kp_launch<K128, 64, false, 51>(a);
+  else if (k <= 32) { if (nb <= 64) kp_launch<u64, 64, false, 0>(a);  else kp_launch<u64, KP_MAX_BUCKETS, false, 0>(a); }
+  else              { if (nb <= 64) kp_launch<K128, 64, false, 0>(a); else kp_launch<K128, KP_MAX_BUCKETS, false, 0>(a); }
   return hipGetLastError();
 }
 
diff --git a/meryl_amd/csrc/mgc_session.hpp b/meryl_amd/csrc/mgc_session.hpp
--- a/meryl_amd/csrc/mgc_session.hpp
+++ b/meryl_amd/csrc/mgc_session.hpp
@@ -84,8 +84,10 @@
   struct Buf { void *p = nullptr; size_t cap = 0; };
   enum { B_PART_WS, B_META, B_X, B_Y, B_SORT_WS, B_RLE_WS, B_UNIQUE, B_COUNTS, B_BLOCKS, B_HPC, B_HPC_WS,
          B_SUBSTART, B_GROUPS, B_GSCAN, B_CNT_TMP, B_LARGE, B_NONEMPTY, B_STAGE0, B_STAGE1, B_TEXT_IN0, B_TEXT_IN1, B_TEXT_WS,
-         B_TEXT_STATE, B_RK, B_RC, B_R2K, B_R2C, B_MERGE_WS, B_SORT_HDRS, B_FINE, B_NARROW_WS, B_Y2, B_Y3, B_Y4, B_HWS0, B_HWS1, B_HWS2, B_HWS3, B_NUM };
+         B_TEXT_STATE, B_RK, B_RC, B_R2K, B_R2C, B_MERGE_WS, B_SORT_HDRS, B_FINE, B_NARROW_WS, B_Y2, B_Y3, B_Y4, B_HWS0, B_HWS1, B_HWS2, B_HWS3,
+         B_PACKED , B_NUM };
   Buf buf[B_NUM];
+  size_t arena_bytes() const { size_t t = 0; for (const auto &b : buf) t += b.cap; return t; }
   double tr_alloc = 0;
   uint64_t tr_alloc_bytes = 0;
   hipError_t ensure(int which, size_t bytes) {
```

Result: faster. 11.90 billion distinct k-mers/s (median of 6 runs) (+1.4%).
